# ChristophReich1996/Semantic_Pyramid_for_Image_Generation

Measured on AMD Instinct MI355X. Metric: images/sec full G+D train step, 256x256, bs/GPU=20, higher is better.
Workload: dtype bf16

## Files before the change

### include/sempyr.h

```cpp
#ifndef SEMPYR_H
#define SEMPYR_H
#include <stdint.h>

#ifdef __cplusplus
extern "C" {
#endif

#define SP_VERSION 1

typedef void* sp_stream_t;

enum sp_status { SP_OK = 0, SP_ERR_INVALID = -1, SP_ERR_LAUNCH = -2, SP_ERR_UNSUPPORTED = -3 };
enum sp_dtype { SP_F32 = 0, SP_BF16 = 1, SP_F8 = 2 ,
                SP_F16 = 3 ,
                SP_F8_F16 = 4  };
enum sp_act { SP_ACT_NONE = 0, SP_ACT_LRELU = 1, SP_ACT_RELU = 2, SP_ACT_TANH = 3 };

int sp_version(void);

enum { SP_TUNE_CONV_TALL = 0, SP_TUNE_IGEMM_DMA = 1, SP_TUNE_WGRAD_ROWS = 2, SP_TUNE_DETERMINISTIC = 3,
       SP_TUNE_SPLITK_TARGET = 4, SP_TUNE_SPLITK_MINSTEPS = 5, SP_TUNE_CONV1X1_DIRECT = 6, SP_TUNE_CONV_SHORT = 7,
       SP_TUNE_WGRAD9_BLOCKS = 8, SP_TUNE_WGRAD_BLOCKS = 9, SP_TUNE_WGRAD_MINSTEPS = 10, SP_TUNE_WGRAD_SMALL_M = 11,
       SP_TUNE_WGRAD_K1_TILE64 = 12, SP_TUNE_WGRAD_ROWS_THIN = 13, SP_TUNE_WGRAD_ROWS_BLOCKS = 14, SP_TUNE_WGRAD_ROWS_SLABS = 15,
       SP_TUNE_CONV_STAGGER = 16, SP_TUNE_CONV1X1_SPLITK = 17, SP_TUNE_WGRAD1X1 = 18, SP_TUNE_CONV_CIN8 = 19, SP_TUNE_CONV_THINCO = 20, SP_TUNE_CONV_PP = 21, SP_TUNE_CONV_PP_PRIO = 22, SP_TUNE_WGRAD_PP = 23, SP_TUNE_BN_ITERS = 24, SP_TUNE_IGEMM_TILE = 25, SP_TUNE_CONV_PPW = 26, SP_TUNE_LINEAR_KS = 27, SP_TUNE_CONV_PP_SPLIT = 28, SP_TUNE_PAIRSET_SEGMENTS = 29, SP_TUNE_COUNT = 30 };
int sp_set_tuning(int32_t key, int32_t value);
const char* sp_last_error_string(void);
const char* sp_last_route(void);

typedef struct sp_conv_params {
    const void* x;
    const void* w;
    const float* bias;
    void* y;
    const void* res1;
    const void* res2;
    const void* mask_src;
    float mask_neg_slope;
    int32_t n, h, w_, cin_p, cout, ldy, ksize, act, dtype;
    void* workspace;
    int64_t workspace_bytes;
    int32_t pool2;
    int32_t in_up2;
    const float* x_scale;
    const float* w_scale;
    void* y8;
    const float* y8_inv_scale;
    float* y8_amax;
    const float* img_scale;
    int32_t img_split;
    int32_t reserved_;
    int64_t split_pix_;
    const void* tail_w;
    const float* tail_bias;
    void* tail_y;
    int32_t tail_cout, tail_act, tail_ld, reserved2_;
    uint32_t* pool_idx;
    int32_t* split_sync;
} sp_conv_params;
#define SP_CONV_SPLIT_SYNC_BYTES 8192
int sp_conv2d_igemm(const sp_conv_params* p, sp_stream_t stream);
int sp_conv2d_workspace(int32_t n, int32_t h, int32_t w_, int32_t cin_p, int32_t cout, int32_t ksize, int32_t dtype,
                        int64_t* bytes_out);
int sp_conv2d_route(const sp_conv_params* p, const char** route);

int sp_conv2d_wgrad(const void* x, const void* dy, float* dw, int32_t n, int32_t h, int32_t w_,
                    int32_t cin_p, int32_t cout, int32_t ld_dy, int32_t ksize, int32_t dtype,
                    sp_stream_t stream);

int sp_conv2d_wgrad_fused(const void* x, const void* dy, float* dw, float* dbias, const void* w_packed, float* dot,
                          float* workspace, int64_t workspace_floats, int32_t n, int32_t h, int32_t w_, int32_t cin_p,
                          int32_t cout, int32_t ld_dy, int32_t ksize, int32_t dtype, sp_stream_t stream);
int sp_conv2d_wgrad_accum(const void* x, const void* dy, float* dw, float* dbias, float* workspace, int64_t workspace_floats,
                          int32_t n, int32_t h, int32_t w_, int32_t cin_p, int32_t cout, int32_t ld_dy, int32_t ksize,
                          int32_t dtype, sp_stream_t stream);
int sp_conv2d_wgrad_accum_pooled(const void* x, const void* dy, float* dw, float* dbias, float* workspace, int64_t workspace_floats,
                                 int32_t n, int32_t h, int32_t w_, int32_t cin_p, int32_t cout, int32_t ld_dy, int32_t ksize,
                                 int32_t dtype, sp_stream_t stream);
int sp_conv2d_wgrad_workspace(int32_t n, int32_t h, int32_t w_, int32_t cin_p, int32_t cout, int32_t ksize,
                              int32_t dtype, int64_t* floats_out);
int sp_conv2d_wgrad_accum_pair(const void* x, const void* dy, float* dw_a, float* dbias_a, float* dw_b, float* dbias_b, float* workspace,
                               int64_t workspace_floats, int32_t n, int32_t split, int32_t h, int32_t w_, int32_t cin_p, int32_t cout,
                               int32_t ld_dy, int32_t ksize, int32_t dy_pooled, int32_t dtype, sp_stream_t stream);
int sp_conv2d_wgrad_route(int32_t n, int32_t split, int32_t h, int32_t w_, int32_t cin_p, int32_t cout, int32_t ld_dy, int32_t ksize,
                          int32_t dy_pooled, int32_t want_dbias, int64_t workspace_floats, int32_t dtype, const char** route);
int sp_wgrad_reduce_defer(int32_t on);
int sp_wgrad_reduce_flush(int32_t run, sp_stream_t stream);
int sp_wgrad_reduce_pending(void);

int sp_linear_fwd(const void* x, int32_t ldx, const void* w_packed, int32_t kp, const float* bias,
                  const void* res, void* y, int32_t ldy, int32_t batch, int32_t k, int32_t n, int32_t act,
                  int32_t dtype, sp_stream_t stream);
int sp_linear_workspace(int32_t batch, int32_t k, int32_t n, int32_t dtype, int64_t* floats_out);
int sp_linear_fwd_ws(const void* x, int32_t ldx, const void* w_packed, int32_t kp, const float* bias,
                     const void* res, void* y, int32_t ldy, int32_t batch, int32_t k, int32_t n, int32_t act,
                     int32_t dtype, float* scratch, sp_stream_t stream);
int sp_linear_wgrad(const void* x, int32_t ldx, const void* dy, int32_t ld_dy, float* dw, int32_t kp,
                    float* dbias, int32_t batch, int32_t k, int32_t n, int32_t dtype, sp_stream_t stream);

typedef struct sp_sn_layer {
    const float* w;
    float* u;
    float* v;
    int64_t scratch_off;
    int64_t part_off;
    int64_t fwd_off;
    int64_t dgrad_off;
    int32_t rows, cols, cin, taps, cin_p, cout_p, kind, pack_block0;
} sp_sn_layer;
int sp_sn_forward(const sp_sn_layer* table_dev, int32_t n_layers, int32_t max_rows, int32_t max_cols,
                  int64_t max_pack_elems, float* scratch, int64_t scratch_floats, void* pack_arena,
                  int32_t power_iter, int32_t dtype, int32_t pack_blocks, sp_stream_t stream);
int sp_sn_pair_scales(const sp_sn_layer* table_dev, int32_t n_layers, const float* scratch_a, const float* scratch_b, float* out,
                      sp_stream_t stream);
typedef struct sp_sn_bwd_layer {
    const float* w;
    int64_t dw_off, dot_off, scratch_off, grad_off;
    int32_t rows, cols, cin, taps, cin_p, plain;
    int32_t db_off, bias_off;
} sp_sn_bwd_layer;
int sp_sn_backward_batched(const sp_sn_bwd_layer* table_dev, int32_t n_layers, int64_t max_elems, float* arena,
                           const float* scratch, float* grads, const float* accumulate_from, float* bias_grads,
                           float* dot_partials, sp_stream_t stream);
int sp_sn_backward_batched_scaled(const sp_sn_bwd_layer* table_dev, int32_t n_layers, int64_t max_elems, float* arena,
                                  const float* scratch, float* grads, const float* accumulate_from, float* bias_grads,
                                  float* dot_partials, float grad_scale, sp_stream_t stream);
int sp_sn_backward_batched_dscaled(const sp_sn_bwd_layer* table_dev, int32_t n_layers, int64_t max_elems, float* arena,
                                   const float* scratch, float* grads, const float* accumulate_from, float* bias_grads,
                                   float* dot_partials, const float* grad_scale_dev, sp_stream_t stream);

int sp_pack_weight(const float* w, int32_t rows, int32_t cols, int32_t cin, int32_t taps, int32_t cin_p,
                   int32_t cout_p, int32_t chw_c, int32_t chw_hw, void* fwd, void* dgrad, int32_t dtype,
                   sp_stream_t stream);
int sp_sn_backward(const float* dwsn, const float* w_orig, const float* layer_scratch, int32_t rows, int32_t cols,
                   int32_t cin, int32_t taps, int32_t cin_p, int32_t plain, float* dot_tmp, int32_t dot_ready,
                   float* grad, sp_stream_t stream);

int sp_bn_stats(const void* x, int32_t n, int64_t hw, int32_t c, float* partials, float eps, float momentum,
                float* running_mean, float* running_var, int32_t training, float* mean_out, float* invstd_out,
                int32_t dtype, sp_stream_t stream);
int sp_bn_apply(const void* x, void* y, int32_t n, int64_t hw, int32_t c, const float* mean, const float* invstd,
                const float* gamma, const float* beta, const float* emb, const int64_t* cls, int32_t act,
                int32_t dtype, sp_stream_t stream);
int sp_bn_stats_pair(const void* x, int32_t n, int32_t split, int64_t hw, int32_t c, float* partials, float eps, float momentum,
                     float* running_mean, float* running_var, int32_t first_group, float* mean2, float* invstd2, int32_t dtype,
                     sp_stream_t stream);
int sp_bn_apply_pair(const void* x, void* y, int32_t n, int32_t split, int64_t hw, int32_t c, const float* mean2, const float* invstd2,
                     const float* gamma, const float* beta, const float* emb, const int64_t* cls, int32_t act, int32_t dtype,
                     sp_stream_t stream);
int sp_bn_apply_upsample2_pair(const void* x, void* y, int32_t n, int32_t split, int32_t h, int32_t w_, int32_t c, const float* mean2,
                               const float* invstd2, const float* gamma, const float* beta, const float* emb, const int64_t* cls,
                               int32_t act, int32_t dtype, sp_stream_t stream);
int sp_bn_apply_upsample2(const void* x, void* y, int32_t n, int32_t h, int32_t w_, int32_t c, const float* mean,
                          const float* invstd, const float* gamma, const float* beta, const float* emb,
                          const int64_t* cls, int32_t act, int32_t dtype, sp_stream_t stream);
int sp_bn_backward(const void* dy, const void* x, void* dx, int32_t n, int64_t hw, int32_t c, const float* mean,
                   const float* invstd, const float* gamma, const float* beta, const float* emb, const int64_t* cls,
                   int32_t act, float* partials, float* c_tmp, float* dgamma, float* dbeta, float* demb,
                   int32_t num_classes, int32_t dtype, sp_stream_t stream);

int sp_bn_stats_up2(const void* x, int32_t n, int32_t h, int32_t w_, int32_t c, float* partials, float eps, float momentum,
                    float* running_mean, float* running_var, float* mean_out, float* invstd_out, int32_t dtype, sp_stream_t stream);
int sp_bn_apply_up2(const void* x, void* y, int32_t n, int32_t h, int32_t w_, int32_t c, const float* mean, const float* invstd,
                    const float* gamma, const float* beta, const float* emb, const int64_t* cls, int32_t act, int32_t dtype,
                    sp_stream_t stream);
int sp_bn_backward_up2(const void* dy, const void* x, void* du, int32_t n, int32_t h, int32_t w_, int32_t c, const float* mean,
                       const float* invstd, const float* gamma, const float* beta, const float* emb, const int64_t* cls,
                       int32_t act, float* partials, float* c_tmp, float* dgamma, float* dbeta, float* demb, int32_t num_classes,
                       int32_t dtype, sp_stream_t stream);

int sp_avgpool2_fwd(const void* x, void* y, void* y_act, int32_t act, int32_t n, int32_t h, int32_t w_, int32_t c,
                    int32_t dtype, sp_stream_t stream);
int sp_avgpool2_bwd(const void* dy, void* dx, int32_t n, int32_t h, int32_t w_, int32_t c, int32_t dtype,
                    sp_stream_t stream);
int sp_act_avgpool2_fwd(const void* x, void* y_act, void* y_pool, int32_t act, int32_t n, int32_t h, int32_t w_, int32_t c,
                        int32_t dtype, sp_stream_t stream);
int sp_act_avgpool2_bwd(const void* d_act, const void* d_pool, const void* x, void* dx, int32_t act, int32_t n, int32_t h,
                        int32_t w_, int32_t c, int32_t dtype, sp_stream_t stream);
int sp_maxpool2_fwd(const void* x, void* y, int32_t n, int32_t h, int32_t w_, int32_t c, int32_t relu, int32_t dtype,
                    sp_stream_t stream);
int sp_maxpool2_bwd(const void* dy, const void* x, void* dx, int32_t n, int32_t h, int32_t w_, int32_t c,
                    int32_t relu, int32_t dtype, sp_stream_t stream);
int sp_maxpool2_bwd_idx(const void* dy, const void* y, const uint32_t* idx, void* dx, int32_t n, int32_t h, int32_t w_, int32_t c,
                        int32_t dtype, sp_stream_t stream);
int sp_adaptive_avgpool_fwd(const void* x, void* y, int32_t n, int32_t h, int32_t w_, int32_t c, int32_t oh,
                            int32_t ow, int32_t act_in, int32_t dtype, sp_stream_t stream);
int sp_adaptive_avgpool_bwd(const void* dy, const void* x, void* dx, int32_t n, int32_t h, int32_t w_, int32_t c,
                            int32_t oh, int32_t ow, int32_t act_in, int32_t dtype, sp_stream_t stream);
int sp_upsample2_fwd(const void* x, void* y, int32_t n, int32_t h, int32_t w_, int32_t c, int32_t dtype,
                     sp_stream_t stream);
int sp_upsample2_bwd(const void* dy, void* dx, int32_t n, int32_t h, int32_t w_, int32_t c, int32_t dtype,
                     sp_stream_t stream);

int sp_attention_bwd_slabs(int32_t n, int32_t nk, int32_t d, int32_t dv, int32_t dtype, int64_t* slabs_out);
int sp_attention_fwd(const void* q, const void* k, const void* v, void* o, float* lse, int32_t batch, int32_t n,
                     int32_t nk, int32_t d, int32_t dv, int32_t dtype, sp_stream_t stream);
int sp_attention_bwd(const void* q, const void* k, const void* v, const void* dout, const float* lse, void* dq,
                     float* dk_f32, float* dv_f32, void* dk, void* dv_out, int32_t batch, int32_t n, int32_t nk,
                     int32_t d, int32_t dv, int32_t dtype, sp_stream_t stream);
int sp_attention_route(int32_t n, int32_t nk, int32_t d, int32_t dv, int32_t dtype, const char** fwd, const char** bwd);

int sp_ingest_image(const void* src, int32_t src_dtype, int64_t sn, int64_t sc, int64_t sh, int64_t sw, void* dst,
                    int32_t n, int32_t c, int32_t h, int32_t w_, int32_t cp, const float* scale3,
                    const float* shift3, int32_t dtype, sp_stream_t stream);
int sp_ingest_image_bwd(const void* dy, int32_t cp, void* dsrc, int32_t c, int64_t pixels, const float* scale3,
                        int32_t dtype, sp_stream_t stream);
enum { SP_AUG_COLOR = 1, SP_AUG_TRANSLATION = 2, SP_AUG_CUTOUT = 4 };
int sp_augment_slices(int32_t h, int32_t w_, int32_t backward, int64_t* slices_out);
int sp_augment_ingest(const void* src, int32_t src_dtype, int64_t sn, int64_t sc, int64_t sh, int64_t sw, void* dst,
                      int32_t n, int32_t h, int32_t w_, int32_t cp, const float* u, int32_t policy, float* partials,
                      int32_t dtype, sp_stream_t stream);
int sp_augment_ingest_bwd(const void* dy, int32_t cp, void* dsrc, int32_t n, int32_t h, int32_t w_, const float* u,
                          int32_t policy, float* partials, int32_t dtype, sp_stream_t stream);
int sp_augment_ingest_gated(const void* src, int32_t src_dtype, int64_t sn, int64_t sc, int64_t sh, int64_t sw, void* dst,
                            int32_t n, int32_t h, int32_t w_, int32_t cp, const float* u, int32_t policy, float* partials,
                            const float* p_dev, int32_t dtype, sp_stream_t stream);
int sp_augment_ingest_bwd_gated(const void* dy, int32_t cp, void* dsrc, int32_t n, int32_t h, int32_t w_, const float* u,
                                int32_t policy, float* partials, const float* p_dev, int32_t dtype, sp_stream_t stream);
int sp_ada_observe(const float* pred, int64_t numel, float threshold, void* state, sp_stream_t stream);
int sp_ada_adjust(void* state, int32_t interval, float target, float step, sp_stream_t stream);
int sp_apa_select(const void* real, int32_t real_dtype, int64_t rn, int64_t rc, int64_t rh, int64_t rw,
                  const void* fake, int32_t fake_dtype, int64_t fn, int64_t fc, int64_t fh, int64_t fw,
                  float* dst, int32_t n, int32_t h, int32_t w_,
                  const float* w_u, const float* p_dev, int32_t dtype, sp_stream_t stream);
enum { SP_GEOM_XFLIP = 1, SP_GEOM_ROT90 = 2, SP_GEOM_SCALE = 4, SP_GEOM_ROTATE = 8 };
int sp_augment_geom_slices(int32_t h, int32_t w_, int32_t backward, int64_t* slices_out);
int sp_augment_geom_decode(const float* u, const float* v, int32_t n, int32_t h, int32_t w_, int32_t policy, int32_t geom,
                           float* table, sp_stream_t stream);
int sp_augment_geom_ingest(const void* src, int32_t src_dtype, int64_t sn, int64_t sc, int64_t sh, int64_t sw, void* dst,
                           int32_t n, int32_t h, int32_t w_, int32_t cp, const float* u, int32_t policy, const float* table,
                           float* partials, const float* p_dev, int32_t dtype, sp_stream_t stream);
int sp_augment_geom_ingest_bwd(const void* dy, int32_t cp, void* dsrc, int32_t n, int32_t h, int32_t w_, const float* u,
                               int32_t policy, const float* table, float* partials, const float* p_dev, int32_t dtype,
                               sp_stream_t stream);
enum { SP_CMAT_BRIGHTNESS = 1, SP_CMAT_CONTRAST = 2, SP_CMAT_LUMAFLIP = 4, SP_CMAT_HUE = 8, SP_CMAT_SATURATION = 16 };
int sp_augment_cmat_decode(const float* z, int32_t n, int32_t cmat, float* ctable, sp_stream_t stream);
int sp_augment_cmat_ingest(const void* src, int32_t src_dtype, int64_t sn, int64_t sc, int64_t sh, int64_t sw, void* dst,
                           int32_t n, int32_t h, int32_t w_, int32_t cp, const float* u, int32_t policy, const float* table,
                           const float* ctable, float* partials, const float* p_dev, int32_t dtype, sp_stream_t stream);
int sp_augment_cmat_ingest_bwd(const void* dy, int32_t cp, void* dsrc, int32_t n, int32_t h, int32_t w_, const float* u,
                               int32_t policy, const float* table, const float* ctable, float* partials, const float* p_dev,
                               int32_t dtype, sp_stream_t stream);
int sp_mask_concat(const void* feat, const float* mask, void* out, int64_t pixels, int32_t c, int32_t cp,
                   int32_t dtype, sp_stream_t stream);
int sp_mask_mul_2d(const void* feat, int32_t ldf, const float* mask, void* out, int32_t ldo, int32_t batch,
                   int32_t k, int32_t dtype, sp_stream_t stream);
int sp_act_fwd(const void* x, void* y, int64_t numel, int32_t act, int32_t dtype, sp_stream_t stream);
int sp_act_bwd(const void* dy, const void* y, void* dz, int64_t pixels, int32_t c, int32_t cp, int32_t act,
               int32_t dtype, sp_stream_t stream);
int sp_scale_add(const void* a, const void* b, const float* g, void* y, int64_t numel, int32_t dtype,
                 sp_stream_t stream);
int sp_rescale_bias(const void* x, void* y, int64_t rows, int32_t c, int32_t ldx, int32_t ldy, const float* bias, const float* sig_a,
                    const float* sig_b, int32_t dtype, sp_stream_t stream);
int sp_scale_add_bwd(const void* dy, const void* a, const float* g, void* da, float* dg, float* partials, int64_t numel,
                     int32_t dtype, sp_stream_t stream);
int sp_permute_chw_hwc(const void* src, void* dst, int32_t batch, int32_t c, int32_t hw, int32_t to_hwc,
                       int32_t dtype, sp_stream_t stream);
int sp_channel_sum(const void* x, int32_t ld, int64_t pixels, int32_t c, float* out, float* partials, int32_t dtype,
                   sp_stream_t stream);
int sp_f64_to_f32(const double* src, float* dst, int32_t n, sp_stream_t stream);

int sp_dhead_fwd(const void* x, int32_t ldx, const float* emb_sn, const int64_t* cls, const float* wc,
                 const float* bc, float* pred, int32_t batch, int32_t f, int32_t dtype, sp_stream_t stream);
int sp_dhead_bwd(const float* dpred, const void* x, int32_t ldx, const float* emb_sn, const int64_t* cls,
                 const float* wc, void* dx, int32_t lddx, float* demb, int32_t num_classes, float* dwc, float* dbc,
                 float* scratch, int32_t batch, int32_t f, int32_t dtype, sp_stream_t stream);
int sp_sqerr_loss_fwd(const float* p, int64_t numel, float target, double* acc_tmp, float* loss, sp_stream_t stream);
int sp_sqerr_loss_bwd(const float* p, int64_t numel, float target, const float* gout, float* dp, sp_stream_t stream);
int sp_rec_loss_fwd(const void* real, int32_t ld_real, const void* fake, int32_t ld_fake, const float* mask,
                    int32_t n, int32_t h, int32_t w_, int32_t c, double* acc, int32_t dtype, sp_stream_t stream);
int sp_rec_loss_bwd(const void* real, int32_t ld_real, const void* fake, int32_t ld_fake, const float* mask,
                    const float* gout, void* dfake, int32_t ld_dfake, int32_t n, int32_t h, int32_t w_, int32_t c,
                    int32_t dtype, sp_stream_t stream);
int sp_div_loss_fwd(const void* img, int64_t half_elems, const float* z, int64_t half_z, double* acc_tmp,
                    float* out2, int32_t dtype, sp_stream_t stream);
int sp_div_loss_bwd(const void* img, int64_t half_elems, const float* fwd_out2, const float* gout, void* dimg,
                    int32_t dtype, sp_stream_t stream);
typedef struct sp_rec_level {
    const void* real; const void* fake; const float* mask;
    void* dfake;
    int32_t ld_real, ld_fake, ld_dfake, n, h, w_, c, reserved_;
} sp_rec_level;
int sp_rec_loss_fwd_levels(const sp_rec_level* levels, int32_t n_levels, double* acc, float* loss, float weight,
                           int32_t dtype, sp_stream_t stream);
int sp_rec_loss_bwd_levels(const sp_rec_level* levels, int32_t n_levels, const float* gout, float weight,
                           int32_t dtype, sp_stream_t stream);
int sp_div_loss_fwd_w(const void* img, int64_t half_elems, const float* z, int64_t half_z, double* acc,
                      float* out2, float weight, int32_t dtype, sp_stream_t stream);

int sp_gan_loss_fwd(const float* p, int64_t numel, int32_t kind, int32_t role, float* loss, sp_stream_t stream);
int sp_gan_loss_bwd(const float* p, int64_t numel, int32_t kind, int32_t role, const float* gout, float* dp, sp_stream_t stream);
int sp_lecam_fwd(const float* pred_real, const float* pred_fake, int64_t numel, float weight, float decay, int32_t start,
                 int32_t rectified, void* state, float* reg, sp_stream_t stream);
int sp_lecam_bwd(const float* pred_real, const float* pred_fake, int64_t numel, float weight, int32_t rectified, const void* state,
                 const float* gout, float* dpred_real, float* dpred_fake, sp_stream_t stream);

int sp_quantize_fp8(const void* x, void* q, int64_t numel, const float* inv_scale, float* amax, int32_t dtype, sp_stream_t stream);
int sp_pack_weight_fp8(const float* w, int32_t cout, int32_t cin, int32_t cin_p, void* out, float* w_scale, sp_stream_t stream);
int sp_fp8_update_scales(float* amax, float* scale, float* inv_scale, int32_t n, float margin, sp_stream_t stream);

int sp_minmax_normalize(const float* x, float* y, int32_t batch, int32_t channels, int64_t hw, float lo, float hi, float eps,
                        int32_t per_channel, sp_stream_t stream);

int sp_training_masks(float* m128, float* m64, float* m32, float* m16, float* m8, float* m4096, float* m365,
                      int32_t batch, uint64_t seed, float p_random_mask, sp_stream_t stream);

typedef struct sp_adam_chunk {
    float* p;
    const float* g;
    float* m;
    float* v;
    int32_t n;
    float step_size;
    float inv_sqrt_bc2;
    float reserved;
} sp_adam_chunk;
int sp_adam_multi(const sp_adam_chunk* chunks_dev, int32_t n_chunks, double beta1, double beta2, double eps,
                  double weight_decay, sp_stream_t stream);

int sp_scale_f32(float* x, int64_t numel, float factor, sp_stream_t stream);
int sp_scale_f32_dev(float* x, int64_t numel, const float* factor_dev, sp_stream_t stream);

int sp_check_finite(const float* x, int64_t numel, float* found, sp_stream_t stream);
int sp_adam_multi_guarded(const sp_adam_chunk* chunks_dev, int32_t n_chunks, double beta1, double beta2, double eps,
                          double weight_decay, const float* skip_if_nonzero, sp_stream_t stream);
int sp_loss_scale_update(float* state, float growth, float backoff, int32_t interval, sp_stream_t stream);

int sp_grad_sqnorm_multi(const sp_adam_chunk* chunks_dev, int32_t n_chunks, double* partials, sp_stream_t stream);
int sp_grad_clip_finalize(const double* partials, int32_t n_partials, double max_norm, float* state, sp_stream_t stream);
int sp_adam_multi_clipped(const sp_adam_chunk* chunks_dev, int32_t n_chunks, double beta1, double beta2, double eps,
                          double weight_decay, const float* skip_if_nonzero, const float* clip_state, sp_stream_t stream);

typedef struct sp_ema_chunk {
    float* avg;
    float* p;
    int32_t n;
    int32_t reserved;
} sp_ema_chunk;
int sp_ema_multi(const sp_ema_chunk* chunks_dev, int32_t n_chunks, float one_minus_decay, const float* skip_if_nonzero,
                 sp_stream_t stream);
int sp_swap_multi(const sp_ema_chunk* chunks_dev, int32_t n_chunks, sp_stream_t stream);

typedef struct sp_conv_general_params {
    int32_t struct_bytes;
    int32_t dtype;
    const void* x;
    const void* w;
    const float* bias;
    void* y;
    int32_t n, h, w_, cin_p, ldx, cout, ldy, kh, kw, stride_h, stride_w, pad_h, pad_w, act;
} sp_conv_general_params;
int sp_conv2d_general(const sp_conv_general_params* p, sp_stream_t stream);
int sp_maxpool3s2_fwd(const void* x, int32_t ldx, void* y, int32_t ldy, int32_t n, int32_t h, int32_t w_, int32_t c, int32_t dtype,
                      sp_stream_t stream);
int sp_avgpool3s1_fwd(const void* x, void* y, int32_t n, int32_t h, int32_t w_, int32_t c, int32_t dtype, sp_stream_t stream);
int sp_inception_prep(const float* x, float* minmax, void* y, int32_t n, int32_t c, int32_t h, int32_t w_, int32_t oh, int32_t ow,
                      int32_t cp, int32_t dtype, sp_stream_t stream);
int sp_global_avgpool_f32(const void* x, float* y, int32_t n, int32_t hw, int32_t c, int32_t dtype, sp_stream_t stream);


int sp_pairset_workspace(int32_t na, int32_t nb, int32_t d, int32_t k, int64_t* bytes);
int sp_pairset_knn(const float* a, int32_t na, int32_t lda, const float* b, int32_t nb, int32_t ldb, int32_t d, int32_t k,
                   int32_t same, float* radius, void* workspace, int64_t workspace_bytes, sp_stream_t stream);
int sp_pairset_cover(const float* a, int32_t na, int32_t lda, const float* b, int32_t nb, int32_t ldb, int32_t d,
                     const float* rad_a, const float* rad_b, int32_t* row_count, int32_t* col_count, float* row_min,
                     float* col_min, void* workspace, int64_t workspace_bytes, sp_stream_t stream);
int sp_pairset_poly3(const float* a, int32_t src_a, int32_t lda, const int32_t* idx_a, const float* b, int32_t src_b, int32_t ldb,
                     const int32_t* idx_b, int32_t d, int32_t subsets, int32_t m, int32_t skip_diag, double* out,
                     void* workspace, int64_t workspace_bytes, sp_stream_t stream);


int sp_pairset_softmax_workspace(int32_t n, int32_t classes, int32_t d, int32_t splits, int64_t* bytes);
int sp_pairset_lse(const float* a, int32_t n, int32_t lda, const float* w, int32_t classes, int32_t ldw, const float* bias, int32_t d,
                   double* lse, double* h, void* workspace, int64_t workspace_bytes, sp_stream_t stream);
int sp_pairset_softmax_colsum(const float* a, int32_t n, int32_t lda, const float* w, int32_t classes, int32_t ldw, const float* bias,
                              int32_t d, const double* lse, const double* h, int32_t splits, double* colsum, double* kl,
                              void* workspace, int64_t workspace_bytes, sp_stream_t stream);

#ifdef __cplusplus
}
#endif
#endif
```

### semantic_pyramid_for_image_generation_amd/_lib.py

```python
from __future__ import annotations

import ctypes
import os
import re
from typing import Dict, List, Tuple

_HERE = os.path.dirname(os.path.abspath(__file__))
HEADER = os.path.join(os.path.dirname(_HERE), "include", "sempyr.h")
LIB_PATH = os.environ.get("SEMPYR_LIB") or os.path.join(_HERE, "libsempyr.so")

SP_F32, SP_BF16, SP_F8, SP_F16, SP_F8_F16 = 0, 1, 2, 3, 4
ACT_NONE, ACT_LRELU, ACT_RELU, ACT_TANH = 0, 1, 2, 3

TUNE_KEYS = {"SP_CONV_TALL": 0, "SP_IGEMM_DMA": 1, "SP_WGRAD_ROWS": 2, "SP_DETERMINISTIC": 3, "SP_SPLITK_TARGET": 4,
             "SP_SPLITK_MINSTEPS": 5, "SP_CONV1X1_DIRECT": 6, "SP_CONV_SHORT": 7, "SP_WGRAD9_BLOCKS": 8, "SP_WGRAD_BLOCKS": 9,
             "SP_WGRAD_MINSTEPS": 10, "SP_WGRAD_SMALL_M": 11, "SP_WGRAD_K1_TILE64": 12, "SP_WGRAD_ROWS_THIN": 13,
             "SP_WGRAD_ROWS_BLOCKS": 14, "SP_WGRAD_ROWS_SLABS": 15, "SP_CONV_STAGGER": 16, "SP_CONV1X1_SPLITK": 17, "SP_WGRAD1X1": 18, "SP_CONV_CIN8": 19, "SP_CONV_THINCO": 20,
             "SP_CONV_PP": 21, "SP_CONV_PP_PRIO": 22, "SP_WGRAD_PP": 23, "SP_BN_ITERS": 24, "SP_IGEMM_TILE": 25, "SP_CONV_PPW": 26, "SP_LINEAR_KS": 27, "SP_CONV_PP_SPLIT": 28, "SP_PAIRSET_SEGMENTS": 29}


SP_CONV_SPLIT_SYNC_BYTES = 8192


class SpConvParams(ctypes.Structure):
    _fields_ = [("x", ctypes.c_void_p), ("w", ctypes.c_void_p), ("bias", ctypes.c_void_p), ("y", ctypes.c_void_p),
                ("res1", ctypes.c_void_p), ("res2", ctypes.c_void_p), ("mask_src", ctypes.c_void_p),
                ("mask_neg_slope", ctypes.c_float),
                ("n", ctypes.c_int32), ("h", ctypes.c_int32), ("w_", ctypes.c_int32), ("cin_p", ctypes.c_int32),
                ("cout", ctypes.c_int32), ("ldy", ctypes.c_int32), ("ksize", ctypes.c_int32), ("act", ctypes.c_int32),
                ("dtype", ctypes.c_int32), ("workspace", ctypes.c_void_p), ("workspace_bytes", ctypes.c_int64),
                ("pool2", ctypes.c_int32), ("in_up2", ctypes.c_int32),
                ("x_scale", ctypes.c_void_p), ("w_scale", ctypes.c_void_p), ("y8", ctypes.c_void_p),
                ("y8_inv_scale", ctypes.c_void_p), ("y8_amax", ctypes.c_void_p),
                ("img_scale", ctypes.c_void_p), ("img_split", ctypes.c_int32), ("reserved_", ctypes.c_int32),
                ("split_pix_", ctypes.c_int64),
                ("tail_w", ctypes.c_void_p), ("tail_bias", ctypes.c_void_p), ("tail_y", ctypes.c_void_p),
                ("tail_cout", ctypes.c_int32), ("tail_act", ctypes.c_int32), ("tail_ld", ctypes.c_int32), ("reserved2_", ctypes.c_int32),
                ("pool_idx", ctypes.c_void_p), ("split_sync", ctypes.c_void_p)]


class SpConvGeneralParams(ctypes.Structure):
    _fields_ = [("struct_bytes", ctypes.c_int32), ("dtype", ctypes.c_int32),
                ("x", ctypes.c_void_p), ("w", ctypes.c_void_p), ("bias", ctypes.c_void_p), ("y", ctypes.c_void_p),
                ("n", ctypes.c_int32), ("h", ctypes.c_int32), ("w_", ctypes.c_int32), ("cin_p", ctypes.c_int32),
                ("ldx", ctypes.c_int32), ("cout", ctypes.c_int32), ("ldy", ctypes.c_int32), ("kh", ctypes.c_int32),
                ("kw", ctypes.c_int32), ("stride_h", ctypes.c_int32), ("stride_w", ctypes.c_int32), ("pad_h", ctypes.c_int32),
                ("pad_w", ctypes.c_int32), ("act", ctypes.c_int32)]

    def __init__(self, **kw):
        super().__init__(struct_bytes=ctypes.sizeof(SpConvGeneralParams), **kw)


class SpSnLayer(ctypes.Structure):
    _fields_ = [("w", ctypes.c_void_p), ("u", ctypes.c_void_p), ("v", ctypes.c_void_p),
                ("scratch_off", ctypes.c_int64), ("part_off", ctypes.c_int64), ("fwd_off", ctypes.c_int64),
                ("dgrad_off", ctypes.c_int64),
                ("rows", ctypes.c_int32), ("cols", ctypes.c_int32), ("cin", ctypes.c_int32), ("taps", ctypes.c_int32),
                ("cin_p", ctypes.c_int32), ("cout_p", ctypes.c_int32), ("kind", ctypes.c_int32),
                ("pack_block0", ctypes.c_int32)]


class SpSnBwdLayer(ctypes.Structure):
    _fields_ = [("w", ctypes.c_void_p), ("dw_off", ctypes.c_int64), ("dot_off", ctypes.c_int64),
                ("scratch_off", ctypes.c_int64), ("grad_off", ctypes.c_int64),
                ("rows", ctypes.c_int32), ("cols", ctypes.c_int32), ("cin", ctypes.c_int32), ("taps", ctypes.c_int32),
                ("cin_p", ctypes.c_int32), ("plain", ctypes.c_int32), ("db_off", ctypes.c_int32),
                ("bias_off", ctypes.c_int32)]


class SpRecLevel(ctypes.Structure):
    _fields_ = [("real", ctypes.c_void_p), ("fake", ctypes.c_void_p), ("mask", ctypes.c_void_p), ("dfake", ctypes.c_void_p),
                ("ld_real", ctypes.c_int32), ("ld_fake", ctypes.c_int32), ("ld_dfake", ctypes.c_int32), ("n", ctypes.c_int32),
                ("h", ctypes.c_int32), ("w_", ctypes.c_int32), ("c", ctypes.c_int32), ("reserved_", ctypes.c_int32)]


_CTYPE = {"int32_t": ctypes.c_int32, "int64_t": ctypes.c_int64, "float": ctypes.c_float, "double": ctypes.c_double, "int": ctypes.c_int,
          "sp_stream_t": ctypes.c_void_p, "uint64_t": ctypes.c_uint64}


def parse_header(path: str = HEADER) -> Dict[str, Tuple[object, List[object]]]:
    text = open(path).read()
    text = re.sub(r"/\*.*?\*/", "", text, flags=re.S)
    protos = {}
    for m in re.finditer(r"\b(int|const char\*)\s+(sp_\w+)\s*\(([^;{]*?)\)\s*;", text, flags=re.S):
        ret, name, args = m.group(1), m.group(2), m.group(3).strip()
        argtypes = []
        if args and args != "void":
            for a in args.split(","):
                a = " ".join(a.split())
                if "*" in a:
                    argtypes.append(ctypes.c_void_p)
                else:
                    ty = a.rsplit(" ", 1)[0].replace("const ", "").strip()
                    argtypes.append(_CTYPE[ty])
        protos[name] = (ctypes.c_char_p if "char" in ret else ctypes.c_int, argtypes)
    return protos


class SempyrError(RuntimeError):
    pass


_lib = None
_protos = None


def lib():
    global _lib, _protos
    if _lib is None:
        if not os.path.exists(LIB_PATH):
            raise SempyrError("libsempyr.so not found at %s - build it with __graft_entry__.build() "
                              "(semantic_pyramid_for_image_generation_amd/csrc/build.sh); there is no fallback path"
                              % LIB_PATH)
        handle = ctypes.CDLL(LIB_PATH)
        _protos = parse_header()
        for name, (ret, argtypes) in _protos.items():
            fn = getattr(handle, name)
            fn.restype = ret
            fn.argtypes = argtypes
        for env_name, key in TUNE_KEYS.items():
            if os.environ.get(env_name) not in (None, ""):
                handle.sp_set_tuning(key, int(os.environ[env_name]))
        _lib = handle
    return _lib


def conv_route(p: SpConvParams) -> str:
    out = ctypes.c_char_p()
    call("sp_conv2d_route", ctypes.byref(p), ctypes.byref(out))
    return out.value.decode()


def wgrad_route(n, split, h, w, cin_p, cout, ld_dy, ksize, dy_pooled, want_dbias, workspace_floats, dtype) -> str:
    out = ctypes.c_char_p()
    call("sp_conv2d_wgrad_route", n, split, h, w, cin_p, cout, ld_dy, ksize, int(dy_pooled), int(want_dbias), workspace_floats, dtype, ctypes.byref(out))
    return out.value.decode()


def attention_route(n, nk, d, dv, dtype):
    fwd, bwd = ctypes.c_char_p(), ctypes.c_char_p()
    call("sp_attention_route", n, nk, d, dv, dtype, ctypes.byref(fwd), ctypes.byref(bwd))
    return fwd.value.decode(), bwd.value.decode()


def call(name: str, *args) -> None:
    rc = getattr(lib(), name)(*args)
    if rc != 0:
        raise SempyrError("%s failed (%d): %s" % (name, rc, lib().sp_last_error_string().decode()))
```

### semantic_pyramid_for_image_generation_amd/csrc/attention.hip

```cpp
#include "common.h"

namespace {


template <typename T, int TQ>
__global__ __launch_bounds__(256) void attn_fwd_kernel(const T* __restrict__ q, const T* __restrict__ k, const T* __restrict__ v,
                                                       T* __restrict__ o, float* __restrict__ lse, int N, int NK, int D, int DV) {
    extern __shared__ __attribute__((aligned(16))) float sm[];
    float* ks = sm;
    float* qs = ks + NK * (D + 1);
    float* S = qs + TQ * D;
    float* vs = S + TQ * NK;
    const int tid = threadIdx.x, lane = tid & 63, wave = tid >> 6;
    const int b = blockIdx.y, q0 = blockIdx.x * TQ;
    const T* kb = k + (long)b * NK * D;
    const T* vb = v + (long)b * NK * DV;
    const T* qb = q + ((long)b * N + q0) * D;
    for (int e = tid; e < NK * D; e += 256) ks[(e / D) * (D + 1) + e % D] = Elem<T>::ld(kb + e);
    for (int e = tid; e < TQ * D; e += 256) qs[e] = (q0 + e / D < N) ? Elem<T>::ld(qb + e) : 0.f;
    __syncthreads();
    for (int j = tid; j < NK; j += 256) {
        const float* kr = ks + j * (D + 1);
        for (int qi = 0; qi < TQ; ++qi) {
            float s = 0.f;
            for (int d = 0; d < D; ++d) s += qs[qi * D + d] * kr[d];
            S[qi * NK + j] = s;
        }
    }
    __syncthreads();
    for (int qi = wave; qi < TQ; qi += 4) {
        float m = -INFINITY;
        for (int j = lane; j < NK; j += 64) m = fmaxf(m, S[qi * NK + j]);
        m = wave_max(m);
        float sum = 0.f;
        for (int j = lane; j < NK; j += 64) { const float e = expf(S[qi * NK + j] - m); S[qi * NK + j] = e; sum += e; }
        sum = wave_sum(sum);
        const float inv = 1.f / sum;
        for (int j = lane; j < NK; j += 64) S[qi * NK + j] *= inv;
        if (lane == 0 && q0 + qi < N) lse[(long)b * N + q0 + qi] = m + logf(sum);
    }
    const int cpar = DV < 256 ? DV : 256;
    const int qpar = 256 / cpar;
    const int qph = tid / cpar;
    const int c = tid % cpar;
    const int nq = (TQ + qpar - 1) / qpar;
    float acc[TQ];
#pragma unroll
    for (int i = 0; i < TQ; ++i) acc[i] = 0.f;
    for (int j0 = 0; j0 < NK; j0 += 32) {
        __syncthreads();
        for (int e = tid; e < 32 * DV; e += 256) vs[e] = (j0 + e / DV < NK) ? Elem<T>::ld(vb + (long)j0 * DV + e) : 0.f;
        __syncthreads();
        if (qph < qpar) {
#pragma unroll 4
            for (int jj = 0; jj < 32; ++jj) {
                const float vv = vs[jj * DV + c];
#pragma unroll
                for (int i = 0; i < TQ; ++i)
                    if (i < nq) acc[i] += S[(qph + i * qpar) * NK + j0 + jj] * vv;
            }
        }
    }
    if (qph < qpar) {
#pragma unroll
        for (int i = 0; i < TQ; ++i) {
            const int qi = qph + i * qpar;
            if (i < nq && qi < TQ && q0 + qi < N) Elem<T>::st(o + ((long)b * N + q0 + qi) * DV + c, acc[i]);
        }
    }
}

template <typename T, int TQ>
__global__ __launch_bounds__(256) void attn_bwd_kernel(const T* __restrict__ q, const T* __restrict__ k, const T* __restrict__ v,
                                                       const T* __restrict__ dout, const float* __restrict__ lse,
                                                       T* __restrict__ dq, float* __restrict__ dk, float* __restrict__ dv,
                                                       int N, int NK, int D, int DV) {
    extern __shared__ __attribute__((aligned(16))) float sm[];
    float* ks = sm;
    float* qs = ks + NK * (D + 1);
    float* dos = qs + TQ * D;
    float* P = dos + TQ * DV;
    float* red = P + TQ * NK;
    float* vt = red + TQ * 4;
    const int tid = threadIdx.x, lane = tid & 63, wave = tid >> 6;
    const int b = blockIdx.y, q0 = blockIdx.x * TQ;
    const T* kb = k + (long)b * NK * D;
    const T* vb = v + (long)b * NK * DV;
    for (int e = tid; e < NK * D; e += 256) ks[(e / D) * (D + 1) + e % D] = Elem<T>::ld(kb + e);
    for (int e = tid; e < TQ * D; e += 256) qs[e] = (q0 + e / D < N) ? Elem<T>::ld(q + ((long)b * N + q0) * D + e) : 0.f;
    for (int e = tid; e < TQ * DV; e += 256) dos[e] = (q0 + e / DV < N) ? Elem<T>::ld(dout + ((long)b * N + q0) * DV + e) : 0.f;
    __syncthreads();
    const int j = tid;
    const bool jl = j < NK;
    float p[TQ], dp[TQ];
#pragma unroll
    for (int qi = 0; qi < TQ; ++qi) { p[qi] = 0.f; dp[qi] = 0.f; }
    if (jl) {
        const float* kr = ks + j * (D + 1);
#pragma unroll
        for (int qi = 0; qi < TQ; ++qi) {
            float s = 0.f;
            for (int d = 0; d < D; ++d) s += qs[qi * D + d] * kr[d];
            p[qi] = (q0 + qi < N) ? expf(s - lse[(long)b * N + q0 + qi]) : 0.f;
        }
    }
    for (int c0 = 0; c0 < DV; c0 += 32) {
        __syncthreads();
        for (int e = tid; e < NK * 32; e += 256) {
            const int jj = e >> 5, cc = e & 31;
            vt[cc * (NK + 1) + jj] = (c0 + cc < DV) ? Elem<T>::ld(vb + (long)jj * DV + c0 + cc) : 0.f;
        }
        __syncthreads();
        if (jl) {
#pragma unroll 4
            for (int cc = 0; cc < 32; ++cc) {
                if (c0 + cc >= DV) break;
                const float vv = vt[cc * (NK + 1) + j];
#pragma unroll
                for (int qi = 0; qi < TQ; ++qi) dp[qi] += dos[qi * DV + c0 + cc] * vv;
            }
        }
    }
    if (jl) {
#pragma unroll
        for (int qi = 0; qi < TQ; ++qi) P[qi * NK + j] = p[qi];
    }
    __syncthreads();
    {
        const int cpar = DV < 256 ? DV : 256, jpar = 256 / cpar;
        const int c = tid % cpar, jph = tid / cpar;
        if (jph < jpar) {
            float dcol[TQ];
#pragma unroll
            for (int qi = 0; qi < TQ; ++qi) dcol[qi] = dos[qi * DV + c];
            for (int jj = jph; jj < NK; jj += jpar) {
                float a = 0.f;
#pragma unroll
                for (int qi = 0; qi < TQ; ++qi) a += P[qi * NK + jj] * dcol[qi];
                dv[((long)blockIdx.x * gridDim.y + b) * NK * DV + (long)jj * DV + c] = a;
            }
        }
    }
#pragma unroll
    for (int qi = 0; qi < TQ; ++qi) {
        const float w = wave_sum(p[qi] * dp[qi]);
        if (lane == 0) red[qi * 4 + wave] = w;
    }
    __syncthreads();
    if (jl) {
#pragma unroll
        for (int qi = 0; qi < TQ; ++qi) {
            const float dr = red[qi * 4] + red[qi * 4 + 1] + red[qi * 4 + 2] + red[qi * 4 + 3];
            const float ds = p[qi] * (dp[qi] - dr);
            P[qi * NK + j] = ds;
            p[qi] = ds;
        }
        for (int d = 0; d < D; ++d) {
            float a = 0.f;
#pragma unroll
            for (int qi = 0; qi < TQ; ++qi) a += p[qi] * qs[qi * D + d];
            dk[((long)blockIdx.x * gridDim.y + b) * NK * D + (long)j * D + d] = a;
        }
    }
    __syncthreads();
    for (int e = tid; e < TQ * D; e += 256) {
        const int qi = e / D, d = e - qi * D;
        float a = 0.f;
        for (int jj = 0; jj < NK; ++jj) a += P[qi * NK + jj] * ks[jj * (D + 1) + d];
        if (q0 + qi < N) Elem<T>::st(dq + ((long)b * N + q0 + qi) * D + d, a);
    }
}


constexpr int AM_NKMAX = 256;
__global__ __launch_bounds__(256) void attn_fwd_mfma_kernel(const bf16* __restrict__ q, const bf16* __restrict__ k,
                                                            const bf16* __restrict__ v, bf16* __restrict__ o, float* __restrict__ lse,
                                                            int N, int NK, int D, int DV) {
    extern __shared__ __attribute__((aligned(16))) char vsm[];
    const int PV = DV * 2 + 32;
    const int tid = threadIdx.x, lane = tid & 63, wave = tid >> 6;
    const int b = blockIdx.y;
    const int q0 = blockIdx.x * 64 + wave * 16;
    const bf16* kb = k + (long)b * NK * D;
    const bf16* vb = v + (long)b * NK * DV;
    const int cpr = DV / 8;
    for (int e = tid; e < NK * cpr; e += 256) {
        const int row = e / cpr, c = e - row * cpr;
        *reinterpret_cast<uint4*>(vsm + row * PV + c * 16) = *reinterpret_cast<const uint4*>(vb + (long)row * DV + c * 8);
    }
    const int i16 = lane & 15, g = lane >> 4;
    const int qrow = min(q0 + i16, N - 1);
    const bf16* qp = q + ((long)b * N + qrow) * D + g * 8;
    f32x4_t sfr[AM_NKMAX / 16];
    const int nf = NK / 16;
#pragma unroll
    for (int f = 0; f < AM_NKMAX / 16; ++f) sfr[f] = f32x4_t{0.f, 0.f, 0.f, 0.f};
    for (int d0 = 0; d0 < D; d0 += 32) {
        const uint4 qv = *reinterpret_cast<const uint4*>(qp + d0);
#pragma unroll
        for (int f = 0; f < AM_NKMAX / 16; ++f) {
            if (f < nf) {
                const uint4 kv = *reinterpret_cast<const uint4*>(kb + (long)(f * 16 + i16) * D + d0 + g * 8);
                sfr[f] = __builtin_amdgcn_mfma_f32_16x16x32_bf16(__builtin_bit_cast(bf16x8_t, kv), __builtin_bit_cast(bf16x8_t, qv), sfr[f], 0, 0, 0);
            }
        }
    }
    float m = -INFINITY;
#pragma unroll
    for (int f = 0; f < AM_NKMAX / 16; ++f)
        if (f < nf) m = fmaxf(fmaxf(fmaxf(m, sfr[f][0]), fmaxf(sfr[f][1], sfr[f][2])), sfr[f][3]);
    m = fmaxf(m, __shfl_xor(m, 16, 64));
    m = fmaxf(m, __shfl_xor(m, 32, 64));
    float sum = 0.f;
#pragma unroll
    for (int f = 0; f < AM_NKMAX / 16; ++f)
        if (f < nf) {
#pragma unroll
            for (int r = 0; r < 4; ++r) { const float e = __expf(sfr[f][r] - m); sfr[f][r] = e; sum += e; }
        }
    sum += __shfl_xor(sum, 16, 64);
    sum += __shfl_xor(sum, 32, 64);
    const float inv = 1.f / sum;
    if (g == 0 && q0 + i16 < N) lse[(long)b * N + q0 + i16] = m + __logf(sum);
    __syncthreads();
    f32x4_t oacc[16];
    const int ncb = DV / 16;
#pragma unroll
    for (int cb = 0; cb < 16; ++cb) oacc[cb] = f32x4_t{0.f, 0.f, 0.f, 0.f};
#pragma unroll
    for (int t = 0; t < AM_NKMAX / 32; ++t) {
        if (t * 32 < NK) {
            uint4 pb;
            pb.x = f32x2_to_bf16x2(sfr[2 * t][0] * inv, sfr[2 * t][1] * inv);
            pb.y = f32x2_to_bf16x2(sfr[2 * t][2] * inv, sfr[2 * t][3] * inv);
            pb.z = f32x2_to_bf16x2(sfr[2 * t + 1][0] * inv, sfr[2 * t + 1][1] * inv);
            pb.w = f32x2_to_bf16x2(sfr[2 * t + 1][2] * inv, sfr[2 * t + 1][3] * inv);
            const char* vrow = vsm + (t * 32 + g * 4 + (i16 >> 2)) * PV + (i16 & 3) * 8;
#pragma unroll
            for (int cb = 0; cb < 16; ++cb) {
                if (cb < ncb) {
                    s16x4_t lo = __builtin_amdgcn_ds_read_tr16_b64_v4i16((__attribute__((address_space(3))) s16x4_t*)(vrow + cb * 32));
                    s16x4_t hi = __builtin_amdgcn_ds_read_tr16_b64_v4i16((__attribute__((address_space(3))) s16x4_t*)(vrow + cb * 32 + 16 * PV));
                    uint2 l2 = __builtin_bit_cast(uint2, lo), h2 = __builtin_bit_cast(uint2, hi);
                    const uint4 va = make_uint4(l2.x, l2.y, h2.x, h2.y);
                    oacc[cb] = __builtin_amdgcn_mfma_f32_16x16x32_bf16(__builtin_bit_cast(bf16x8_t, va), __builtin_bit_cast(bf16x8_t, pb), oacc[cb], 0, 0, 0);
                }
            }
        }
    }
    if (q0 + i16 < N) {
        bf16* op = o + ((long)b * N + q0 + i16) * DV + g * 4;
#pragma unroll
        for (int cb = 0; cb < 16; ++cb)
            if (cb < ncb) {
                const float t4[4] = {oacc[cb][0], oacc[cb][1], oacc[cb][2], oacc[cb][3]};
                Elem<bf16>::st4(op + cb * 16, t4);
            }
    }
}

constexpr int AB_QB = 64;
__device__ __forceinline__ uint4 tr_pair(const char* p, int hi_off) {
    s16x4_t lo = __builtin_amdgcn_ds_read_tr16_b64_v4i16((__attribute__((address_space(3))) s16x4_t*)(p));
    s16x4_t hi = __builtin_amdgcn_ds_read_tr16_b64_v4i16((__attribute__((address_space(3))) s16x4_t*)(p + hi_off));
    const uint2 l2 = __builtin_bit_cast(uint2, lo), h2 = __builtin_bit_cast(uint2, hi);
    return make_uint4(l2.x, l2.y, h2.x, h2.y);
}
__device__ __forceinline__ uint4 pack8(const f32x4_t& a, const f32x4_t& b) {
    uint4 r;
    r.x = f32x2_to_bf16x2(a[0], a[1]);
    r.y = f32x2_to_bf16x2(a[2], a[3]);
    r.z = f32x2_to_bf16x2(b[0], b[1]);
    r.w = f32x2_to_bf16x2(b[2], b[3]);
    return r;
}

__global__ __launch_bounds__(256) void attn_bwd_mfma_kernel(const bf16* __restrict__ q, const bf16* __restrict__ k,
                                                            const bf16* __restrict__ v, const bf16* __restrict__ dout,
                                                            const float* __restrict__ lse, bf16* __restrict__ dq,
                                                            float* __restrict__ dk, float* __restrict__ dv, int N, int NK, int D, int DV) {
    extern __shared__ __attribute__((aligned(16))) char bsm[];
    const int PK = D * 2 + 32, PDO = DV * 2 + 32, PP = NK * 2 + 32;
    char* Ksm = bsm;
    char* Qsm = Ksm + NK * PK;
    char* dOsm = Qsm + AB_QB * PK;
    char* Psm = dOsm + AB_QB * PDO;
    char* dSsm = Psm + AB_QB * PP;
    const int PVL = DV * 2 + 16;
    const bool v_in_lds = NK * PVL <= 2 * AB_QB * PP;
    const int tid = threadIdx.x, lane = tid & 63, wave = tid >> 6;
    const int b = blockIdx.y, qb0 = blockIdx.x * AB_QB;
    const bf16* kb = k + (long)b * NK * D;
    const bf16* vb = v + (long)b * NK * DV;
    float* dk_slab = dk + (long)blockIdx.x * gridDim.y * NK * D;
    float* dv_slab = dv + (long)blockIdx.x * gridDim.y * NK * DV;
    {
        const int cpr = D / 8;
        for (int e = tid; e < NK * cpr; e += 256) {
            const int row = e / cpr, c = e - row * cpr;
            *reinterpret_cast<uint4*>(Ksm + row * PK + c * 16) = *reinterpret_cast<const uint4*>(kb + (long)row * D + c * 8);
        }
        for (int e = tid; e < AB_QB * cpr; e += 256) {
            const int row = e / cpr, c = e - row * cpr;
            uint4 val = make_uint4(0, 0, 0, 0);
            if (qb0 + row < N) val = *reinterpret_cast<const uint4*>(q + ((long)b * N + qb0 + row) * D + c * 8);
            *reinterpret_cast<uint4*>(Qsm + row * PK + c * 16) = val;
        }
        const int cpo = DV / 8;
        for (int e = tid; e < AB_QB * cpo; e += 256) {
            const int row = e / cpo, c = e - row * cpo;
            uint4 val = make_uint4(0, 0, 0, 0);
            if (qb0 + row < N) val = *reinterpret_cast<const uint4*>(dout + ((long)b * N + qb0 + row) * DV + c * 8);
            *reinterpret_cast<uint4*>(dOsm + row * PDO + c * 16) = val;
        }
        if (v_in_lds) {
            for (int e = tid; e < NK * cpo; e += 256) {
                const int row = e / cpo, c = e - row * cpo;
                *reinterpret_cast<uint4*>(Psm + row * PVL + c * 16) = *reinterpret_cast<const uint4*>(vb + (long)row * DV + c * 8);
            }
        }
    }
    __syncthreads();
    const int i16 = lane & 15, g = lane >> 4;
    const int ql = wave * 16 + i16;
    const bool q_ok = qb0 + ql < N;
    const int nf = NK / 16;
    f32x4_t pfr[AM_NKMAX / 16], dpf[AM_NKMAX / 16];
#pragma unroll
    for (int f = 0; f < AM_NKMAX / 16; ++f) { pfr[f] = f32x4_t{0.f, 0.f, 0.f, 0.f}; dpf[f] = f32x4_t{0.f, 0.f, 0.f, 0.f}; }
    for (int d0 = 0; d0 < D; d0 += 32) {
        const uint4 qv = *reinterpret_cast<const uint4*>(Qsm + ql * PK + (d0 + g * 8) * 2);
#pragma unroll
        for (int f = 0; f < AM_NKMAX / 16; ++f)
            if (f < nf) {
                const uint4 kv = *reinterpret_cast<const uint4*>(Ksm + (f * 16 + i16) * PK + (d0 + g * 8) * 2);
                pfr[f] = __builtin_amdgcn_mfma_f32_16x16x32_bf16(__builtin_bit_cast(bf16x8_t, kv), __builtin_bit_cast(bf16x8_t, qv), pfr[f], 0, 0, 0);
            }
    }
    for (int c0 = 0; c0 < DV; c0 += 32) {
        const uint4 dov = *reinterpret_cast<const uint4*>(dOsm + ql * PDO + (c0 + g * 8) * 2);
#pragma unroll
        for (int f = 0; f < AM_NKMAX / 16; ++f)
            if (f < nf) {
                const uint4 vv = v_in_lds ? *reinterpret_cast<const uint4*>(Psm + (f * 16 + i16) * PVL + (c0 + g * 8) * 2)
                                          : *reinterpret_cast<const uint4*>(vb + (long)(f * 16 + i16) * DV + c0 + g * 8);
                dpf[f] = __builtin_amdgcn_mfma_f32_16x16x32_bf16(__builtin_bit_cast(bf16x8_t, vv), __builtin_bit_cast(bf16x8_t, dov), dpf[f], 0, 0, 0);
            }
    }
    const float l = q_ok ? lse[(long)b * N + qb0 + ql] : 0.f;
    float drow = 0.f;
#pragma unroll
    for (int f = 0; f < AM_NKMAX / 16; ++f)
        if (f < nf) {
#pragma unroll
            for (int r = 0; r < 4; ++r) {
                const float pv = q_ok ? __expf(pfr[f][r] - l) : 0.f;
                pfr[f][r] = pv;
                drow += pv * dpf[f][r];
            }
        }
    drow += __shfl_xor(drow, 16, 64);
    drow += __shfl_xor(drow, 32, 64);
#pragma unroll
    for (int f = 0; f < AM_NKMAX / 16; ++f)
        if (f < nf) {
#pragma unroll
            for (int r = 0; r < 4; ++r) dpf[f][r] = pfr[f][r] * (dpf[f][r] - drow);
        }
    {
        f32x4_t dqa[4];
        const int ndb = D / 16;
#pragma unroll
        for (int db = 0; db < 4; ++db) dqa[db] = f32x4_t{0.f, 0.f, 0.f, 0.f};
#pragma unroll
        for (int t = 0; t < AM_NKMAX / 32; ++t)
            if (t * 32 < NK) {
                const uint4 sb = pack8(dpf[2 * t], dpf[2 * t + 1]);
                const char* krow = Ksm + (t * 32 + g * 4 + (i16 >> 2)) * PK + (i16 & 3) * 8;
#pragma unroll
                for (int db = 0; db < 4; ++db)
                    if (db < ndb) {
                        const uint4 ka = tr_pair(krow + db * 32, 16 * PK);
                        dqa[db] = __builtin_amdgcn_mfma_f32_16x16x32_bf16(__builtin_bit_cast(bf16x8_t, ka), __builtin_bit_cast(bf16x8_t, sb), dqa[db], 0, 0, 0);
                    }
            }
        if (q_ok) {
            bf16* qp = dq + ((long)b * N + qb0 + ql) * D + g * 4;
#pragma unroll
            for (int db = 0; db < 4; ++db)
                if (db < ndb) {
                    const float t4[4] = {dqa[db][0], dqa[db][1], dqa[db][2], dqa[db][3]};
                    Elem<bf16>::st4(qp + db * 16, t4);
                }
        }
    }
    if (v_in_lds) __syncthreads();
#pragma unroll
    for (int f = 0; f < AM_NKMAX / 16; ++f)
        if (f < nf) {
            uint2 pw, sw;
            pw.x = f32x2_to_bf16x2(pfr[f][0], pfr[f][1]);
            pw.y = f32x2_to_bf16x2(pfr[f][2], pfr[f][3]);
            sw.x = f32x2_to_bf16x2(dpf[f][0], dpf[f][1]);
            sw.y = f32x2_to_bf16x2(dpf[f][2], dpf[f][3]);
            *reinterpret_cast<uint2*>(Psm + ql * PP + (f * 16 + g * 4) * 2) = pw;
            *reinterpret_cast<uint2*>(dSsm + ql * PP + (f * 16 + g * 4) * 2) = sw;
        }
    __syncthreads();
    const int rowsel = g * 4 + (i16 >> 2), colsel = (i16 & 3) * 8;
    for (int cb0 = 0; cb0 < DV / 16; cb0 += 8) {
        f32x4_t acc[4][8];
        const int ncb = min(8, DV / 16 - cb0);
#pragma unroll
        for (int a = 0; a < 4; ++a)
#pragma unroll
            for (int cb = 0; cb < 8; ++cb) acc[a][cb] = f32x4_t{0.f, 0.f, 0.f, 0.f};
#pragma unroll
        for (int t2 = 0; t2 < AB_QB / 32; ++t2) {
            uint4 pb[4];
#pragma unroll
            for (int a = 0; a < 4; ++a) {
                const int kf = wave + 4 * a;
                pb[a] = tr_pair(Psm + (t2 * 32 + rowsel) * PP + colsel + (kf < nf ? kf : 0) * 32, 16 * PP);
            }
#pragma unroll
            for (int cb = 0; cb < 8; ++cb)
                if (cb < ncb) {
                    const uint4 da = tr_pair(dOsm + (t2 * 32 + rowsel) * PDO + colsel + (cb0 + cb) * 32, 16 * PDO);
#pragma unroll
                    for (int a = 0; a < 4; ++a)
                        acc[a][cb] = __builtin_amdgcn_mfma_f32_16x16x32_bf16(__builtin_bit_cast(bf16x8_t, da), __builtin_bit_cast(bf16x8_t, pb[a]), acc[a][cb], 0, 0, 0);
                }
        }
#pragma unroll
        for (int a = 0; a < 4; ++a) {
            const int kf = wave + 4 * a;
            if (kf < nf) {
                float* dst = dv_slab + ((long)b * NK + kf * 16 + i16) * DV + cb0 * 16 + g * 4;
#pragma unroll
                for (int cb = 0; cb < 8; ++cb)
                    if (cb < ncb) *reinterpret_cast<float4*>(dst + cb * 16) = make_float4(acc[a][cb][0], acc[a][cb][1], acc[a][cb][2], acc[a][cb][3]);
            }
        }
    }
    {
        f32x4_t acc[4][4];
        const int ndb = D / 16;
#pragma unroll
        for (int a = 0; a < 4; ++a)
#pragma unroll
            for (int db = 0; db < 4; ++db) acc[a][db] = f32x4_t{0.f, 0.f, 0.f, 0.f};
#pragma unroll
        for (int t2 = 0; t2 < AB_QB / 32; ++t2) {
            uint4 sb[4];
#pragma unroll
            for (int a = 0; a < 4; ++a) {
                const int kf = wave + 4 * a;
                sb[a] = tr_pair(dSsm + (t2 * 32 + rowsel) * PP + colsel + (kf < nf ? kf : 0) * 32, 16 * PP);
            }
#pragma unroll
            for (int db = 0; db < 4; ++db)
                if (db < ndb) {
                    const uint4 qa = tr_pair(Qsm + (t2 * 32 + rowsel) * PK + colsel + db * 32, 16 * PK);
#pragma unroll
                    for (int a = 0; a < 4; ++a)
                        acc[a][db] = __builtin_amdgcn_mfma_f32_16x16x32_bf16(__builtin_bit_cast(bf16x8_t, qa), __builtin_bit_cast(bf16x8_t, sb[a]), acc[a][db], 0, 0, 0);
                }
        }
#pragma unroll
        for (int a = 0; a < 4; ++a) {
            const int kf = wave + 4 * a;
            if (kf < nf) {
                float* dst = dk_slab + ((long)b * NK + kf * 16 + i16) * D + g * 4;
#pragma unroll
                for (int db = 0; db < 4; ++db)
                    if (db < ndb) *reinterpret_cast<float4*>(dst + db * 16) = make_float4(acc[a][db][0], acc[a][db][1], acc[a][db][2], acc[a][db][3]);
            }
        }
    }
}

template <typename T>
__global__ void attn_reduce_kernel(const float* __restrict__ src, int nslabs, long n, T* __restrict__ dst) {
    for (long i = (long)blockIdx.x * 256 + threadIdx.x; i < n / 4; i += (long)gridDim.x * 256) {
        float4 a = reinterpret_cast<const float4*>(src)[i];
        for (int s = 1; s < nslabs; ++s) {
            const float4 t = reinterpret_cast<const float4*>(src + (long)s * n)[i];
            a.x += t.x; a.y += t.y; a.z += t.z; a.w += t.w;
        }
        const float o[4] = {a.x, a.y, a.z, a.w};
        Elem<T>::st4(dst + i * 4, o);
    }
}

template <typename T>
__global__ void cast_f32_kernel(const float* __restrict__ src, T* __restrict__ dst, long n) {
    for (long i = (long)blockIdx.x * 256 + threadIdx.x; i < n; i += (long)gridDim.x * 256) Elem<T>::st(dst + i, src[i]);
}

template <typename T, int TQ>
int launch_attn_tq(bool fwd, const void* q, const void* k, const void* v, void* o_or_dq, const void* dout, float* lse, float* dk,
                   float* dv, int B, int N, int NK, int D, int DV, hipStream_t s) {
    const int lds_f = (NK * (D + 1) + TQ * D + TQ * NK + 32 * DV) * 4;
    const int lds_b = (NK * (D + 1) + TQ * D + TQ * DV + TQ * NK + TQ * 4 + 32 * (NK + 1)) * 4;
    dim3 grid(sp_div_up(N, TQ), B);
    if (fwd) {
        if (const int rc = sp_lds_limit<attn_fwd_kernel<T, TQ>>(lds_f)) return rc;
        hipLaunchKernelGGL((attn_fwd_kernel<T, TQ>), grid, dim3(256), lds_f, s, (const T*)q, (const T*)k, (const T*)v, (T*)o_or_dq, lse, N, NK, D, DV);
    } else {
        if (const int rc = sp_lds_limit<attn_bwd_kernel<T, TQ>>(lds_b)) return rc;
        hipLaunchKernelGGL((attn_bwd_kernel<T, TQ>), grid, dim3(256), lds_b, s, (const T*)q, (const T*)k, (const T*)v, (const T*)dout, lse,
                           (T*)o_or_dq, dk, dv, N, NK, D, DV);
    }
    SP_LAUNCH_CHECK();
    return SP_OK;
}

inline int attn_valu_tq(int NK, int D, int DV) {
    const long lds_b32 = (long)(NK * (D + 1) + 32 * D + 32 * DV + 32 * NK + 32 * 4 + 32 * (NK + 1)) * 4;
    return lds_b32 <= 160 * 1024 ? 32 : 16;
}
inline bool attn_fwd_mfma_ok(int dtype, int nk, int d, int dv) {
    return dtype == SP_BF16 && d % 32 == 0 && dv % 16 == 0 && dv <= 256 && nk % 32 == 0;
}
inline bool attn_bwd_mfma_ok(int dtype, int nk, int d, int dv) {
    return dtype == SP_BF16 && (d == 32 || d == 64) && dv % 32 == 0 && dv <= 256 && nk % 32 == 0;
}
inline const char* attn_valu_name(int nk, int d, int dv) { return attn_valu_tq(nk, d, dv) == 32 ? "valu tq32" : "valu tq16"; }
template <typename T>
int launch_attn(bool fwd, const void* q, const void* k, const void* v, void* o_or_dq, const void* dout, float* lse, float* dk,
                float* dv, int B, int N, int NK, int D, int DV, hipStream_t s) {
    if (attn_valu_tq(NK, D, DV) == 32) return launch_attn_tq<T, 32>(fwd, q, k, v, o_or_dq, dout, lse, dk, dv, B, N, NK, D, DV, s);
    return launch_attn_tq<T, 16>(fwd, q, k, v, o_or_dq, dout, lse, dk, dv, B, N, NK, D, DV, s);
}

}

extern "C" int sp_attention_fwd(const void* q, const void* k, const void* v, void* o, float* lse, int32_t batch, int32_t n,
                                int32_t nk, int32_t d, int32_t dv, int32_t dtype, sp_stream_t stream) {
    SP_CHECK_ARG(q && k && v && o && lse, "sp_attention_fwd: null pointer");
    SP_CHECK_ARG(nk > 0 && nk <= 256 && d > 0 && d <= 64 && dv > 0 && dv <= 256, "sp_attention_fwd: unsupported extents nk=%d d=%d dv=%d", nk, d, dv);
    hipStream_t s = reinterpret_cast<hipStream_t>(stream);
    if (attn_fwd_mfma_ok(dtype, nk, d, dv)) {
        const int lds = nk * (dv * 2 + 32);
        if (const int rc = sp_lds_limit<attn_fwd_mfma_kernel>(lds)) return rc;
        hipLaunchKernelGGL(attn_fwd_mfma_kernel, dim3(sp_div_up(n, 64), batch), dim3(256), lds, s, (const bf16*)q, (const bf16*)k, (const bf16*)v,
                           (bf16*)o, lse, n, nk, d, dv);
        SP_LAUNCH_CHECK();
        return SP_OK;
    }
    return dtype == SP_F32 ? launch_attn<float>(true, q, k, v, o, nullptr, lse, nullptr, nullptr, batch, n, nk, d, dv, s)
                           : launch_attn<bf16>(true, q, k, v, o, nullptr, lse, nullptr, nullptr, batch, n, nk, d, dv, s);
}

extern "C" int sp_attention_bwd(const void* q, const void* k, const void* v, const void* dout, const float* lse, void* dq,
                                float* dk_f32, float* dv_f32, void* dk, void* dv_out, int32_t batch, int32_t n, int32_t nk,
                                int32_t d, int32_t dv, int32_t dtype, sp_stream_t stream) {
    SP_CHECK_ARG(q && k && v && dout && lse && dq && dk_f32 && dv_f32 && dk && dv_out, "sp_attention_bwd: null pointer");
    SP_CHECK_ARG(nk > 0 && nk <= 256 && d > 0 && d <= 64 && dv > 0 && dv <= 256, "sp_attention_bwd: unsupported extents nk=%d d=%d dv=%d", nk, d, dv);
    hipStream_t s = reinterpret_cast<hipStream_t>(stream);
    const long nkd = (long)batch * nk * d, nkv = (long)batch * nk * dv;
    if (attn_bwd_mfma_ok(dtype, nk, d, dv)) {
        const int nqb = sp_div_up(n, AB_QB);
        const int lds = nk * (d * 2 + 32) + AB_QB * (d * 2 + 32) + AB_QB * (dv * 2 + 32) + 2 * AB_QB * (nk * 2 + 32);
        if (const int rc = sp_lds_limit<attn_bwd_mfma_kernel>(lds)) return rc;
        hipLaunchKernelGGL(attn_bwd_mfma_kernel, dim3(nqb, batch), dim3(256), lds, s, (const bf16*)q, (const bf16*)k,
                           (const bf16*)v, (const bf16*)dout, lse, (bf16*)dq, dk_f32, dv_f32, n, nk, d, dv);
        hipLaunchKernelGGL(attn_reduce_kernel<bf16>, dim3(sp_div_up(nkd / 4, 256)), dim3(256), 0, s, dk_f32, nqb, nkd, (bf16*)dk);
        hipLaunchKernelGGL(attn_reduce_kernel<bf16>, dim3(sp_div_up(nkv / 4, 256)), dim3(256), 0, s, dv_f32, nqb, nkv, (bf16*)dv_out);
        SP_LAUNCH_CHECK();
        return SP_OK;
    }
    SP_CHECK_ARG(nkd % 4 == 0 && nkv % 4 == 0, "sp_attention_bwd: batch*nk*d and batch*nk*dv must be multiples of 4");
    const int nqb = sp_div_up(n, attn_valu_tq(nk, d, dv));
    int rc = dtype == SP_F32 ? launch_attn<float>(false, q, k, v, dq, dout, const_cast<float*>(lse), dk_f32, dv_f32, batch, n, nk, d, dv, s)
                             : launch_attn<bf16>(false, q, k, v, dq, dout, const_cast<float*>(lse), dk_f32, dv_f32, batch, n, nk, d, dv, s);
    if (rc != SP_OK) return rc;
    if (dtype == SP_F32) {
        hipLaunchKernelGGL(attn_reduce_kernel<float>, dim3(sp_div_up(nkd / 4, 256)), dim3(256), 0, s, dk_f32, nqb, nkd, (float*)dk);
        hipLaunchKernelGGL(attn_reduce_kernel<float>, dim3(sp_div_up(nkv / 4, 256)), dim3(256), 0, s, dv_f32, nqb, nkv, (float*)dv_out);
    } else {
        hipLaunchKernelGGL(attn_reduce_kernel<bf16>, dim3(sp_div_up(nkd / 4, 256)), dim3(256), 0, s, dk_f32, nqb, nkd, (bf16*)dk);
        hipLaunchKernelGGL(attn_reduce_kernel<bf16>, dim3(sp_div_up(nkv / 4, 256)), dim3(256), 0, s, dv_f32, nqb, nkv, (bf16*)dv_out);
    }
    SP_LAUNCH_CHECK();
    return SP_OK;
}

extern "C" int sp_attention_bwd_slabs(int32_t n, int32_t nk, int32_t d, int32_t dv, int32_t dtype, int64_t* slabs_out) {
    SP_CHECK_ARG(slabs_out && n > 0 && nk > 0 && d > 0 && dv > 0, "sp_attention_bwd_slabs: bad args");
    *slabs_out = attn_bwd_mfma_ok(dtype, nk, d, dv) ? sp_div_up(n, AB_QB) : sp_div_up(n, attn_valu_tq(nk, d, dv));
    return SP_OK;
}

extern "C" int sp_attention_route(int32_t n, int32_t nk, int32_t d, int32_t dv, int32_t dtype, const char** fwd, const char** bwd) {
    SP_CHECK_ARG(fwd != nullptr && bwd != nullptr, "sp_attention_route: null argument");
    SP_CHECK_ARG(dtype == SP_F32 || dtype == SP_BF16, "sp_attention_route: unsupported storage type %d", dtype);
    SP_CHECK_ARG(n > 0 && nk > 0 && nk <= 256 && d > 0 && d <= 64 && dv > 0 && dv <= 256, "sp_attention_route: unsupported extents n=%d nk=%d d=%d dv=%d", n, nk, d, dv);
    *fwd = attn_fwd_mfma_ok(dtype, nk, d, dv) ? "mfma" : attn_valu_name(nk, d, dv);
    *bwd = attn_bwd_mfma_ok(dtype, nk, d, dv) ? "mfma" : attn_valu_name(nk, d, dv);
    return SP_OK;
}
```

Before: 1322.

## Make attention blocks walk several query tiles, keeping K/V resident across tiles

The forward attention kernel now loops over several 64-row query tiles per block. K stays in registers when d=32 and V is staged into LDS once per block, so it is reused across tiles instead of reloaded per tile. A new backward kernel keeps K and V resident in LDS while walking query tiles, which cuts the number of fp32 dK/dV slabs. The two slab reductions are merged into one launch. The walk length is derived from the CU count and can be overridden by a new tuning key. Fewer blocks means less parallelism for small batches, and a cycle-counter timing variant of the old backward kernel is added behind a tuning flag.

Result: faster. 1339, median of 6 (+1.3%).

```diff
diff --git a/include/sempyr.h b/include/sempyr.h
--- a/include/sempyr.h
+++ b/include/sempyr.h
@@ -22,7 +22,7 @@
        SP_TUNE_SPLITK_TARGET = 4, SP_TUNE_SPLITK_MINSTEPS = 5, SP_TUNE_CONV1X1_DIRECT = 6, SP_TUNE_CONV_SHORT = 7,
        SP_TUNE_WGRAD9_BLOCKS = 8, SP_TUNE_WGRAD_BLOCKS = 9, SP_TUNE_WGRAD_MINSTEPS = 10, SP_TUNE_WGRAD_SMALL_M = 11,
        SP_TUNE_WGRAD_K1_TILE64 = 12, SP_TUNE_WGRAD_ROWS_THIN = 13, SP_TUNE_WGRAD_ROWS_BLOCKS = 14, SP_TUNE_WGRAD_ROWS_SLABS = 15,
-       SP_TUNE_CONV_STAGGER = 16, SP_TUNE_CONV1X1_SPLITK = 17, SP_TUNE_WGRAD1X1 = 18, SP_TUNE_CONV_CIN8 = 19, SP_TUNE_CONV_THINCO = 20, SP_TUNE_CONV_PP = 21, SP_TUNE_CONV_PP_PRIO = 22, SP_TUNE_WGRAD_PP = 23, SP_TUNE_BN_ITERS = 24, SP_TUNE_IGEMM_TILE = 25, SP_TUNE_CONV_PPW = 26, SP_TUNE_LINEAR_KS = 27, SP_TUNE_CONV_PP_SPLIT = 28, SP_TUNE_PAIRSET_SEGMENTS = 29, SP_TUNE_COUNT = 30 };
+       SP_TUNE_CONV_STAGGER = 16, SP_TUNE_CONV1X1_SPLITK = 17, SP_TUNE_WGRAD1X1 = 18, SP_TUNE_CONV_CIN8 = 19, SP_TUNE_CONV_THINCO = 20, SP_TUNE_CONV_PP = 21, SP_TUNE_CONV_PP_PRIO = 22, SP_TUNE_WGRAD_PP = 23, SP_TUNE_BN_ITERS = 24, SP_TUNE_IGEMM_TILE = 25, SP_TUNE_CONV_PPW = 26, SP_TUNE_LINEAR_KS = 27, SP_TUNE_CONV_PP_SPLIT = 28, SP_TUNE_PAIRSET_SEGMENTS = 29, SP_TUNE_ATTN_PIECES = 30, SP_TUNE_COUNT = 31 };
 int sp_set_tuning(int32_t key, int32_t value);
 const char* sp_last_error_string(void);
 const char* sp_last_route(void);
@@ -198,6 +198,8 @@
                      float* dk_f32, float* dv_f32, void* dk, void* dv_out, int32_t batch, int32_t n, int32_t nk,
                      int32_t d, int32_t dv, int32_t dtype, sp_stream_t stream);
 int sp_attention_route(int32_t n, int32_t nk, int32_t d, int32_t dv, int32_t dtype, const char** fwd, const char** bwd);
+int sp_attention_plan(int32_t batch, int32_t n, int32_t nk, int32_t d, int32_t dv, int32_t dtype, int32_t cus,
+                      int32_t* fwd_walk, int32_t* bwd_walk, int32_t* bwd_slabs);
 
 int sp_ingest_image(const void* src, int32_t src_dtype, int64_t sn, int64_t sc, int64_t sh, int64_t sw, void* dst,
                     int32_t n, int32_t c, int32_t h, int32_t w_, int32_t cp, const float* scale3,
diff --git a/semantic_pyramid_for_image_generation_amd/_lib.py b/semantic_pyramid_for_image_generation_amd/_lib.py
--- a/semantic_pyramid_for_image_generation_amd/_lib.py
+++ b/semantic_pyramid_for_image_generation_amd/_lib.py
@@ -16,7 +16,7 @@
              "SP_SPLITK_MINSTEPS": 5, "SP_CONV1X1_DIRECT": 6, "SP_CONV_SHORT": 7, "SP_WGRAD9_BLOCKS": 8, "SP_WGRAD_BLOCKS": 9,
              "SP_WGRAD_MINSTEPS": 10, "SP_WGRAD_SMALL_M": 11, "SP_WGRAD_K1_TILE64": 12, "SP_WGRAD_ROWS_THIN": 13,
              "SP_WGRAD_ROWS_BLOCKS": 14, "SP_WGRAD_ROWS_SLABS": 15, "SP_CONV_STAGGER": 16, "SP_CONV1X1_SPLITK": 17, "SP_WGRAD1X1": 18, "SP_CONV_CIN8": 19, "SP_CONV_THINCO": 20,
-             "SP_CONV_PP": 21, "SP_CONV_PP_PRIO": 22, "SP_WGRAD_PP": 23, "SP_BN_ITERS": 24, "SP_IGEMM_TILE": 25, "SP_CONV_PPW": 26, "SP_LINEAR_KS": 27, "SP_CONV_PP_SPLIT": 28, "SP_PAIRSET_SEGMENTS": 29}
+             "SP_CONV_PP": 21, "SP_CONV_PP_PRIO": 22, "SP_WGRAD_PP": 23, "SP_BN_ITERS": 24, "SP_IGEMM_TILE": 25, "SP_CONV_PPW": 26, "SP_LINEAR_KS": 27, "SP_CONV_PP_SPLIT": 28, "SP_PAIRSET_SEGMENTS": 29, "SP_ATTN_PIECES": 30}
 
 
 SP_CONV_SPLIT_SYNC_BYTES = 8192
diff --git a/semantic_pyramid_for_image_generation_amd/csrc/attention.hip b/semantic_pyramid_for_image_generation_amd/csrc/attention.hip
--- a/semantic_pyramid_for_image_generation_amd/csrc/attention.hip
+++ b/semantic_pyramid_for_image_generation_amd/csrc/attention.hip
@@ -173,93 +173,146 @@
 
 
 constexpr int AM_NKMAX = 256;
-__global__ __launch_bounds__(256) void attn_fwd_mfma_kernel(const bf16* __restrict__ q, const bf16* __restrict__ k,
-                                                            const bf16* __restrict__ v, bf16* __restrict__ o, float* __restrict__ lse,
-                                                            int N, int NK, int D, int DV) {
+constexpr int AB_QB = 64;
+
+template <int BATCH>
+__device__ __forceinline__ void stage_chunks(char* dst, int pitch, const bf16* __restrict__ src, int chunks, int live, int cpr, int tid) {
+    const uint4* s4 = reinterpret_cast<const uint4*>(src);
+    for (int e0 = tid; e0 < chunks; e0 += 256 * BATCH) {
+        uint4 r[BATCH];
+#pragma unroll
+        for (int i = 0; i < BATCH; ++i) r[i] = s4[min(e0 + i * 256, live - 1)];
+#pragma unroll
+        for (int i = 0; i < BATCH; ++i) {
+            const int e = e0 + i * 256;
+            if (e < chunks) {
+                const int row = e / cpr, c = e - row * cpr;
+                *reinterpret_cast<uint4*>(dst + row * pitch + c * 16) = e < live ? r[i] : make_uint4(0, 0, 0, 0);
+            }
+        }
+    }
+}
+
+constexpr int ATTN_TIMING_BIT = 4096;
+inline int attn_walk(int batch, int nqb, int slots, int pieces) {
+    if (pieces >= ATTN_TIMING_BIT) pieces = -1;
+    if (pieces >= 0) return sp_div_up(nqb, pieces < 1 ? 1 : pieces > nqb ? nqb : pieces);
+    int r = 1;
+    while (r < nqb && (long)batch * sp_div_up(nqb, r) > slots) ++r;
+    return r;
+}
+inline int attn_cus() {
+    static const int cus = [] {
+        int dev = 0, n = 0;
+        if (hipGetDevice(&dev) != hipSuccess || hipDeviceGetAttribute(&n, hipDeviceAttributeMultiprocessorCount, dev) != hipSuccess || n <= 0) {
+            (void)hipGetLastError();
+            n = 256;
+        }
+        return n;
+    }();
+    return cus;
+}
+inline int attn_fwd_lds(int nk, int dv) { return nk * (dv * 2 + 32); }
+inline int attn_fwd_slots(int cus, int nk, int dv) { return 2 * attn_fwd_lds(nk, dv) <= 160 * 1024 ? 2 * cus : cus; }
+
+template <bool KREG>
+__global__ __launch_bounds__(256, 2) void attn_fwd_mfma_kernel(const bf16* __restrict__ q, const bf16* __restrict__ k,
+                                                               const bf16* __restrict__ v, bf16* __restrict__ o, float* __restrict__ lse,
+                                                               int N, int NK, int D, int DV, int R) {
     extern __shared__ __attribute__((aligned(16))) char vsm[];
     const int PV = DV * 2 + 32;
     const int tid = threadIdx.x, lane = tid & 63, wave = tid >> 6;
     const int b = blockIdx.y;
-    const int q0 = blockIdx.x * 64 + wave * 16;
+    const int nqb = (N + AB_QB - 1) / AB_QB;
+    const int blk0 = blockIdx.x * R, nit = min(R, nqb - blk0);
     const bf16* kb = k + (long)b * NK * D;
     const bf16* vb = v + (long)b * NK * DV;
-    const int cpr = DV / 8;
-    for (int e = tid; e < NK * cpr; e += 256) {
-        const int row = e / cpr, c = e - row * cpr;
-        *reinterpret_cast<uint4*>(vsm + row * PV + c * 16) = *reinterpret_cast<const uint4*>(vb + (long)row * DV + c * 8);
-    }
     const int i16 = lane & 15, g = lane >> 4;
-    const int qrow = min(q0 + i16, N - 1);
-    const bf16* qp = q + ((long)b * N + qrow) * D + g * 8;
-    f32x4_t sfr[AM_NKMAX / 16];
     const int nf = NK / 16;
-#pragma unroll
-    for (int f = 0; f < AM_NKMAX / 16; ++f) sfr[f] = f32x4_t{0.f, 0.f, 0.f, 0.f};
-    for (int d0 = 0; d0 < D; d0 += 32) {
-        const uint4 qv = *reinterpret_cast<const uint4*>(qp + d0);
-#pragma unroll
-        for (int f = 0; f < AM_NKMAX / 16; ++f) {
+    const bf16* qimg = q + (long)b * N * D + g * 8;
+    uint4 qv0 = *reinterpret_cast<const uint4*>(qimg + (long)min(blk0 * AB_QB + wave * 16 + i16, N - 1) * D);
+    uint4 kfr[KREG ? AM_NKMAX / 16 : 1];
+    if constexpr (KREG) {
+#pragma unroll
+        for (int f = 0; f < AM_NKMAX / 16; ++f)
+            kfr[f] = *reinterpret_cast<const uint4*>(kb + (long)(min(f, nf - 1) * 16 + i16) * D + g * 8);
+    }
+    stage_chunks<8>(vsm, PV, vb, NK * (DV / 8), NK * (DV / 8), DV / 8, tid);
+    __syncthreads();
+    for (int it = 0; it < nit; ++it) {
+        const int q0 = (blk0 + it) * AB_QB + wave * 16;
+        const int qrow = min(q0 + i16, N - 1);
+        uint4 qv = qv0;
+        if (it + 1 < nit) qv0 = *reinterpret_cast<const uint4*>(qimg + (long)min(q0 + AB_QB + i16, N - 1) * D);
+        f32x4_t sfr[AM_NKMAX / 16];
+#pragma unroll
+        for (int f = 0; f < AM_NKMAX / 16; ++f) sfr[f] = f32x4_t{0.f, 0.f, 0.f, 0.f};
+        for (int d0 = 0; d0 < D; d0 += 32) {
+            if (d0 > 0) qv = *reinterpret_cast<const uint4*>(qimg + (long)qrow * D + d0);
+#pragma unroll
+            for (int f = 0; f < AM_NKMAX / 16; ++f) {
+                if (f < nf) {
+                    uint4 kv;
+                    if constexpr (KREG) kv = kfr[f];
+                    else kv = *reinterpret_cast<const uint4*>(kb + (long)(f * 16 + i16) * D + d0 + g * 8);
+                    sfr[f] = __builtin_amdgcn_mfma_f32_16x16x32_bf16(__builtin_bit_cast(bf16x8_t, kv), __builtin_bit_cast(bf16x8_t, qv), sfr[f], 0, 0, 0);
+                }
+            }
+        }
+        float m = -INFINITY;
+#pragma unroll
+        for (int f = 0; f < AM_NKMAX / 16; ++f)
+            if (f < nf) m = fmaxf(fmaxf(fmaxf(m, sfr[f][0]), fmaxf(sfr[f][1], sfr[f][2])), sfr[f][3]);
+        m = fmaxf(m, __shfl_xor(m, 16, 64));
+        m = fmaxf(m, __shfl_xor(m, 32, 64));
+        float sum = 0.f;
+#pragma unroll
+        for (int f = 0; f < AM_NKMAX / 16; ++f)
             if (f < nf) {
-                const uint4 kv = *reinterpret_cast<const uint4*>(kb + (long)(f * 16 + i16) * D + d0 + g * 8);
-                sfr[f] = __builtin_amdgcn_mfma_f32_16x16x32_bf16(__builtin_bit_cast(bf16x8_t, kv), __builtin_bit_cast(bf16x8_t, qv), sfr[f], 0, 0, 0);
-            }
-        }
-    }
-    float m = -INFINITY;
-#pragma unroll
-    for (int f = 0; f < AM_NKMAX / 16; ++f)
-        if (f < nf) m = fmaxf(fmaxf(fmaxf(m, sfr[f][0]), fmaxf(sfr[f][1], sfr[f][2])), sfr[f][3]);
-    m = fmaxf(m, __shfl_xor(m, 16, 64));
-    m = fmaxf(m, __shfl_xor(m, 32, 64));
-    float sum = 0.f;
-#pragma unroll
-    for (int f = 0; f < AM_NKMAX / 16; ++f)
-        if (f < nf) {
-#pragma unroll
-            for (int r = 0; r < 4; ++r) { const float e = __expf(sfr[f][r] - m); sfr[f][r] = e; sum += e; }
-        }
-    sum += __shfl_xor(sum, 16, 64);
-    sum += __shfl_xor(sum, 32, 64);
-    const float inv = 1.f / sum;
-    if (g == 0 && q0 + i16 < N) lse[(long)b * N + q0 + i16] = m + __logf(sum);
-    __syncthreads();
-    f32x4_t oacc[16];
-    const int ncb = DV / 16;
-#pragma unroll
-    for (int cb = 0; cb < 16; ++cb) oacc[cb] = f32x4_t{0.f, 0.f, 0.f, 0.f};
-#pragma unroll
-    for (int t = 0; t < AM_NKMAX / 32; ++t) {
-        if (t * 32 < NK) {
-            uint4 pb;
-            pb.x = f32x2_to_bf16x2(sfr[2 * t][0] * inv, sfr[2 * t][1] * inv);
-            pb.y = f32x2_to_bf16x2(sfr[2 * t][2] * inv, sfr[2 * t][3] * inv);
-            pb.z = f32x2_to_bf16x2(sfr[2 * t + 1][0] * inv, sfr[2 * t + 1][1] * inv);
-            pb.w = f32x2_to_bf16x2(sfr[2 * t + 1][2] * inv, sfr[2 * t + 1][3] * inv);
-            const char* vrow = vsm + (t * 32 + g * 4 + (i16 >> 2)) * PV + (i16 & 3) * 8;
-#pragma unroll
-            for (int cb = 0; cb < 16; ++cb) {
+#pragma unroll
+                for (int r = 0; r < 4; ++r) { const float e = __expf(sfr[f][r] - m); sfr[f][r] = e; sum += e; }
+            }
+        sum += __shfl_xor(sum, 16, 64);
+        sum += __shfl_xor(sum, 32, 64);
+        const float inv = 1.f / sum;
+        if (g == 0 && q0 + i16 < N) lse[(long)b * N + q0 + i16] = m + __logf(sum);
+        f32x4_t oacc[16];
+        const int ncb = DV / 16;
+#pragma unroll
+        for (int cb = 0; cb < 16; ++cb) oacc[cb] = f32x4_t{0.f, 0.f, 0.f, 0.f};
+#pragma unroll
+        for (int t = 0; t < AM_NKMAX / 32; ++t) {
+            if (t * 32 < NK) {
+                uint4 pb;
+                pb.x = f32x2_to_bf16x2(sfr[2 * t][0] * inv, sfr[2 * t][1] * inv);
+                pb.y = f32x2_to_bf16x2(sfr[2 * t][2] * inv, sfr[2 * t][3] * inv);
+                pb.z = f32x2_to_bf16x2(sfr[2 * t + 1][0] * inv, sfr[2 * t + 1][1] * inv);
+                pb.w = f32x2_to_bf16x2(sfr[2 * t + 1][2] * inv, sfr[2 * t + 1][3] * inv);
+                const char* vrow = vsm + (t * 32 + g * 4 + (i16 >> 2)) * PV + (i16 & 3) * 8;
+#pragma unroll
+                for (int cb = 0; cb < 16; ++cb) {
+                    if (cb < ncb) {
+                        s16x4_t lo = __builtin_amdgcn_ds_read_tr16_b64_v4i16((__attribute__((address_space(3))) s16x4_t*)(vrow + cb * 32));
+                        s16x4_t hi = __builtin_amdgcn_ds_read_tr16_b64_v4i16((__attribute__((address_space(3))) s16x4_t*)(vrow + cb * 32 + 16 * PV));
+                        uint2 l2 = __builtin_bit_cast(uint2, lo), h2 = __builtin_bit_cast(uint2, hi);
+                        const uint4 va = make_uint4(l2.x, l2.y, h2.x, h2.y);
+                        oacc[cb] = __builtin_amdgcn_mfma_f32_16x16x32_bf16(__builtin_bit_cast(bf16x8_t, va), __builtin_bit_cast(bf16x8_t, pb), oacc[cb], 0, 0, 0);
+                    }
+                }
+            }
+        }
+        if (q0 + i16 < N) {
+            bf16* op = o + ((long)b * N + q0 + i16) * DV + g * 4;
+#pragma unroll
+            for (int cb = 0; cb < 16; ++cb)
                 if (cb < ncb) {
-                    s16x4_t lo = __builtin_amdgcn_ds_read_tr16_b64_v4i16((__attribute__((address_space(3))) s16x4_t*)(vrow + cb * 32));
-                    s16x4_t hi = __builtin_amdgcn_ds_read_tr16_b64_v4i16((__attribute__((address_space(3))) s16x4_t*)(vrow + cb * 32 + 16 * PV));
-                    uint2 l2 = __builtin_bit_cast(uint2, lo), h2 = __builtin_bit_cast(uint2, hi);
-                    const uint4 va = make_uint4(l2.x, l2.y, h2.x, h2.y);
-                    oacc[cb] = __builtin_amdgcn_mfma_f32_16x16x32_bf16(__builtin_bit_cast(bf16x8_t, va), __builtin_bit_cast(bf16x8_t, pb), oacc[cb], 0, 0, 0);
-                }
-            }
-        }
-    }
-    if (q0 + i16 < N) {
-        bf16* op = o + ((long)b * N + q0 + i16) * DV + g * 4;
-#pragma unroll
-        for (int cb = 0; cb < 16; ++cb)
-            if (cb < ncb) {
-                const float t4[4] = {oacc[cb][0], oacc[cb][1], oacc[cb][2], oacc[cb][3]};
-                Elem<bf16>::st4(op + cb * 16, t4);
-            }
-    }
-}
-
-constexpr int AB_QB = 64;
+                    const float t4[4] = {oacc[cb][0], oacc[cb][1], oacc[cb][2], oacc[cb][3]};
+                    Elem<bf16>::st4(op + cb * 16, t4);
+                }
+        }
+    }
+}
+
 __device__ __forceinline__ uint4 tr_pair(const char* p, int hi_off) {
     s16x4_t lo = __builtin_amdgcn_ds_read_tr16_b64_v4i16((__attribute__((address_space(3))) s16x4_t*)(p));
     s16x4_t hi = __builtin_amdgcn_ds_read_tr16_b64_v4i16((__attribute__((address_space(3))) s16x4_t*)(p + hi_off));
@@ -275,6 +328,7 @@
     return r;
 }
 
+template <bool TIMING = false>
 __global__ __launch_bounds__(256) void attn_bwd_mfma_kernel(const bf16* __restrict__ q, const bf16* __restrict__ k,
                                                             const bf16* __restrict__ v, const bf16* __restrict__ dout,
                                                             const float* __restrict__ lse, bf16* __restrict__ dq,
@@ -294,6 +348,16 @@
     const bf16* vb = v + (long)b * NK * DV;
     float* dk_slab = dk + (long)blockIdx.x * gridDim.y * NK * D;
     float* dv_slab = dv + (long)blockIdx.x * gridDim.y * NK * DV;
+    unsigned long long tacc[6] = {0, 0, 0, 0, 0, 0};
+    unsigned long long tprev = 0;
+    auto stamp = [&](int i) {
+        if constexpr (TIMING) {
+            const unsigned long long t = __builtin_readcyclecounter();
+            tacc[i] += t - tprev;
+            tprev = t;
+        }
+    };
+    if constexpr (TIMING) tprev = __builtin_readcyclecounter();
     {
         const int cpr = D / 8;
         for (int e = tid; e < NK * cpr; e += 256) {
@@ -321,6 +385,7 @@
         }
     }
     __syncthreads();
+    stamp(0);
     const int i16 = lane & 15, g = lane >> 4;
     const int ql = wave * 16 + i16;
     const bool q_ok = qb0 + ql < N;
@@ -367,6 +432,7 @@
 #pragma unroll
             for (int r = 0; r < 4; ++r) dpf[f][r] = pfr[f][r] * (dpf[f][r] - drow);
         }
+    stamp(1);
     {
         f32x4_t dqa[4];
         const int ndb = D / 16;
@@ -394,6 +460,7 @@
                 }
         }
     }
+    stamp(2);
     if (v_in_lds) __syncthreads();
 #pragma unroll
     for (int f = 0; f < AM_NKMAX / 16; ++f)
@@ -407,6 +474,7 @@
             *reinterpret_cast<uint2*>(dSsm + ql * PP + (f * 16 + g * 4) * 2) = sw;
         }
     __syncthreads();
+    stamp(3);
     const int rowsel = g * 4 + (i16 >> 2), colsel = (i16 & 3) * 8;
     for (int cb0 = 0; cb0 < DV / 16; cb0 += 8) {
         f32x4_t acc[4][8];
@@ -443,6 +511,7 @@
             }
         }
     }
+    stamp(4);
     {
         f32x4_t acc[4][4];
         const int ndb = D / 16;
@@ -478,6 +547,241 @@
             }
         }
     }
+    if constexpr (TIMING) {
+        stamp(5);
+        __syncthreads();
+        if (lane == 0)
+            for (int i = 0; i < 6; ++i) dk_slab[(long)b * NK * D + wave * 8 + i] = (float)tacc[i];
+    }
+}
+
+inline int attn_bwd_res_lds(int nk, int d, int dv) {
+    return nk * (d * 2 + 32) + nk * (dv * 2 + 16) + AB_QB * (d * 2 + 32) + AB_QB * (dv * 2 + 32) + 2 * (AB_QB / 2) * (nk * 2 + 32);
+}
+inline bool attn_bwd_res_ok(int nk, int d, int dv) { return d == 32 && dv <= 128 && attn_bwd_res_lds(nk, d, dv) <= 160 * 1024; }
+
+__global__ __launch_bounds__(256) void attn_bwd_res_kernel(const bf16* __restrict__ q, const bf16* __restrict__ k,
+                                                           const bf16* __restrict__ v, const bf16* __restrict__ dout,
+                                                           const float* __restrict__ lse, bf16* __restrict__ dq,
+                                                           float* __restrict__ dk, float* __restrict__ dv, int N, int NK, int DV, int R) {
+    extern __shared__ __attribute__((aligned(16))) char bsm[];
+    constexpr int D = 32, ND = D / 32, PK = D * 2 + 32, HQ = AB_QB / 2, NDB = D / 16;
+    const int PDO = DV * 2 + 32, PP = NK * 2 + 32, PVL = DV * 2 + 16;
+    char* Ksm = bsm;
+    char* Vsm = Ksm + NK * PK;
+    char* Qsm = Vsm + NK * PVL;
+    char* dOsm = Qsm + AB_QB * PK;
+    char* Psm = dOsm + AB_QB * PDO;
+    char* dSsm = Psm + HQ * PP;
+    const int tid = threadIdx.x, lane = tid & 63, wave = tid >> 6;
+    const int b = blockIdx.y;
+    const int nqb = (N + AB_QB - 1) / AB_QB;
+    const int blk0 = blockIdx.x * R, nit = min(R, nqb - blk0);
+    const int i16 = lane & 15, g = lane >> 4;
+    const int ql = wave * 16 + i16;
+    const int nf = NK / 16, ncb = DV / 16;
+    const int cpq = D / 8, cpo = DV / 8;
+    const bf16* qimg = q + (long)b * N * D;
+    const bf16* doimg = dout + (long)b * N * DV;
+    const float* limg = lse + (long)b * N;
+    float l_cur = limg[min(blk0 * AB_QB + ql, N - 1)];
+    {
+        const int live = min(AB_QB, N - blk0 * AB_QB);
+        stage_chunks<8>(Ksm, PK, k + (long)b * NK * D, NK * cpq, NK * cpq, cpq, tid);
+        stage_chunks<8>(Vsm, PVL, v + (long)b * NK * DV, NK * cpo, NK * cpo, cpo, tid);
+        stage_chunks<ND>(Qsm, PK, qimg + (long)blk0 * AB_QB * D, AB_QB * cpq, live * cpq, cpq, tid);
+        stage_chunks<4>(dOsm, PDO, doimg + (long)blk0 * AB_QB * DV, AB_QB * cpo, live * cpo, cpo, tid);
+    }
+    f32x4_t accv[4][8], acck[4][NDB];
+#pragma unroll
+    for (int a = 0; a < 4; ++a) {
+#pragma unroll
+        for (int cb = 0; cb < 8; ++cb) accv[a][cb] = f32x4_t{0.f, 0.f, 0.f, 0.f};
+#pragma unroll
+        for (int db = 0; db < NDB; ++db) acck[a][db] = f32x4_t{0.f, 0.f, 0.f, 0.f};
+    }
+    const int rowsel = g * 4 + (i16 >> 2), colsel = (i16 & 3) * 8;
+    auto contract = [&](int h) {
+        uint4 pb[4], sb[4];
+#pragma unroll
+        for (int a = 0; a < 4; ++a) {
+            const int kf = wave + 4 * a, off = rowsel * PP + colsel + (kf < nf ? kf : 0) * 32;
+            pb[a] = tr_pair(Psm + off, 16 * PP);
+            sb[a] = tr_pair(dSsm + off, 16 * PP);
+        }
+#pragma unroll
+        for (int cb = 0; cb < 8; ++cb)
+            if (cb < ncb) {
+                const uint4 da = tr_pair(dOsm + (h * HQ + rowsel) * PDO + colsel + cb * 32, 16 * PDO);
+#pragma unroll
+                for (int a = 0; a < 4; ++a)
+                    accv[a][cb] = __builtin_amdgcn_mfma_f32_16x16x32_bf16(__builtin_bit_cast(bf16x8_t, da), __builtin_bit_cast(bf16x8_t, pb[a]), accv[a][cb], 0, 0, 0);
+            }
+#pragma unroll
+        for (int db = 0; db < NDB; ++db) {
+            const uint4 qa = tr_pair(Qsm + (h * HQ + rowsel) * PK + colsel + db * 32, 16 * PK);
+#pragma unroll
+            for (int a = 0; a < 4; ++a)
+                acck[a][db] = __builtin_amdgcn_mfma_f32_16x16x32_bf16(__builtin_bit_cast(bf16x8_t, qa), __builtin_bit_cast(bf16x8_t, sb[a]), acck[a][db], 0, 0, 0);
+        }
+    };
+    for (int it = 0; it < nit; ++it) {
+        const int qb0 = (blk0 + it) * AB_QB;
+        const bool q_ok = qb0 + ql < N;
+        __syncthreads();
+        f32x4_t pfr[AM_NKMAX / 16], dpf[AM_NKMAX / 16];
+#pragma unroll
+        for (int f = 0; f < AM_NKMAX / 16; ++f) { pfr[f] = f32x4_t{0.f, 0.f, 0.f, 0.f}; dpf[f] = f32x4_t{0.f, 0.f, 0.f, 0.f}; }
+#pragma unroll
+        for (int d0 = 0; d0 < D; d0 += 32) {
+            const uint4 qv = *reinterpret_cast<const uint4*>(Qsm + ql * PK + (d0 + g * 8) * 2);
+#pragma unroll
+            for (int f = 0; f < AM_NKMAX / 16; ++f)
+                if (f < nf) {
+                    const uint4 kv = *reinterpret_cast<const uint4*>(Ksm + (f * 16 + i16) * PK + (d0 + g * 8) * 2);
+                    pfr[f] = __builtin_amdgcn_mfma_f32_16x16x32_bf16(__builtin_bit_cast(bf16x8_t, kv), __builtin_bit_cast(bf16x8_t, qv), pfr[f], 0, 0, 0);
+                }
+        }
+        for (int c0 = 0; c0 < DV; c0 += 32) {
+            const uint4 dov = *reinterpret_cast<const uint4*>(dOsm + ql * PDO + (c0 + g * 8) * 2);
+#pragma unroll
+            for (int f = 0; f < AM_NKMAX / 16; ++f)
+                if (f < nf) {
+                    const uint4 vv = *reinterpret_cast<const uint4*>(Vsm + (f * 16 + i16) * PVL + (c0 + g * 8) * 2);
+                    dpf[f] = __builtin_amdgcn_mfma_f32_16x16x32_bf16(__builtin_bit_cast(bf16x8_t, vv), __builtin_bit_cast(bf16x8_t, dov), dpf[f], 0, 0, 0);
+                }
+        }
+        const float l = q_ok ? l_cur : 0.f;
+        float drow = 0.f;
+#pragma unroll
+        for (int f = 0; f < AM_NKMAX / 16; ++f)
+            if (f < nf) {
+#pragma unroll
+                for (int r = 0; r < 4; ++r) {
+                    const float pv = q_ok ? __expf(pfr[f][r] - l) : 0.f;
+                    pfr[f][r] = pv;
+                    drow += pv * dpf[f][r];
+                }
+            }
+        drow += __shfl_xor(drow, 16, 64);
+        drow += __shfl_xor(drow, 32, 64);
+        uint2 pw[AM_NKMAX / 16], sw[AM_NKMAX / 16];
+#pragma unroll
+        for (int f = 0; f < AM_NKMAX / 16; ++f) {
+            pw[f] = make_uint2(0, 0);
+            sw[f] = make_uint2(0, 0);
+            if (f < nf) {
+                pw[f].x = f32x2_to_bf16x2(pfr[f][0], pfr[f][1]);
+                pw[f].y = f32x2_to_bf16x2(pfr[f][2], pfr[f][3]);
+                sw[f].x = f32x2_to_bf16x2(pfr[f][0] * (dpf[f][0] - drow), pfr[f][1] * (dpf[f][1] - drow));
+                sw[f].y = f32x2_to_bf16x2(pfr[f][2] * (dpf[f][2] - drow), pfr[f][3] * (dpf[f][3] - drow));
+            }
+        }
+        {
+            f32x4_t dqa[NDB];
+#pragma unroll
+            for (int db = 0; db < NDB; ++db) dqa[db] = f32x4_t{0.f, 0.f, 0.f, 0.f};
+#pragma unroll
+            for (int t = 0; t < AM_NKMAX / 32; ++t)
+                if (t * 32 < NK) {
+                    const uint4 sb = make_uint4(sw[2 * t].x, sw[2 * t].y, sw[2 * t + 1].x, sw[2 * t + 1].y);
+                    const char* krow = Ksm + (t * 32 + g * 4 + (i16 >> 2)) * PK + (i16 & 3) * 8;
+#pragma unroll
+                    for (int db = 0; db < NDB; ++db) {
+                        const uint4 ka = tr_pair(krow + db * 32, 16 * PK);
+                        dqa[db] = __builtin_amdgcn_mfma_f32_16x16x32_bf16(__builtin_bit_cast(bf16x8_t, ka), __builtin_bit_cast(bf16x8_t, sb), dqa[db], 0, 0, 0);
+                    }
+                }
+            if (q_ok) {
+                bf16* qp = dq + ((long)b * N + qb0 + ql) * D + g * 4;
+#pragma unroll
+                for (int db = 0; db < NDB; ++db) {
+                    const float t4[4] = {dqa[db][0], dqa[db][1], dqa[db][2], dqa[db][3]};
+                    Elem<bf16>::st4(qp + db * 16, t4);
+                }
+            }
+        }
+        const bool more = it + 1 < nit;
+        const int live = more ? min(AB_QB, N - qb0 - AB_QB) : 1;
+        uint4 qn[ND], don[4];
+        float l_next = 0.f;
+        if (more) {
+            const uint4* q4 = reinterpret_cast<const uint4*>(qimg + (long)(qb0 + AB_QB) * D);
+            const uint4* o4 = reinterpret_cast<const uint4*>(doimg + (long)(qb0 + AB_QB) * DV);
+#pragma unroll
+            for (int i = 0; i < ND; ++i) qn[i] = q4[min(tid + i * 256, live * cpq - 1)];
+#pragma unroll
+            for (int i = 0; i < 4; ++i) don[i] = o4[min(tid + i * 256, live * cpo - 1)];
+            l_next = limg[min(qb0 + AB_QB + ql, N - 1)];
+        }
+        auto put = [&](int row) {
+#pragma unroll
+            for (int f = 0; f < AM_NKMAX / 16; ++f)
+                if (f < nf) {
+                    *reinterpret_cast<uint2*>(Psm + row * PP + (f * 16 + g * 4) * 2) = pw[f];
+                    *reinterpret_cast<uint2*>(dSsm + row * PP + (f * 16 + g * 4) * 2) = sw[f];
+                }
+        };
+        if (wave < 2) put(ql);
+        __syncthreads();
+        contract(0);
+        __syncthreads();
+        if (wave >= 2) put(ql - HQ);
+        __syncthreads();
+        contract(1);
+        if (more) {
+            __syncthreads();
+#pragma unroll
+            for (int i = 0; i < ND; ++i) {
+                const int e = tid + i * 256, row = e / cpq, c = e - row * cpq;
+                *reinterpret_cast<uint4*>(Qsm + row * PK + c * 16) = e < live * cpq ? qn[i] : make_uint4(0, 0, 0, 0);
+            }
+#pragma unroll
+            for (int i = 0; i < 4; ++i) {
+                const int e = tid + i * 256, row = e / cpo, c = e - row * cpo;
+                if (e < AB_QB * cpo) *reinterpret_cast<uint4*>(dOsm + row * PDO + c * 16) = e < live * cpo ? don[i] : make_uint4(0, 0, 0, 0);
+            }
+            l_cur = l_next;
+        }
+    }
+    float* dk_slab = dk + ((long)blockIdx.x * gridDim.y + b) * NK * D;
+    float* dv_slab = dv + ((long)blockIdx.x * gridDim.y + b) * NK * DV;
+#pragma unroll
+    for (int a = 0; a < 4; ++a) {
+        const int kf = wave + 4 * a;
+        if (kf < nf) {
+            float* dst = dv_slab + (long)(kf * 16 + i16) * DV + g * 4;
+#pragma unroll
+            for (int cb = 0; cb < 8; ++cb)
+                if (cb < ncb) *reinterpret_cast<float4*>(dst + cb * 16) = make_float4(accv[a][cb][0], accv[a][cb][1], accv[a][cb][2], accv[a][cb][3]);
+            dst = dk_slab + (long)(kf * 16 + i16) * D + g * 4;
+#pragma unroll
+            for (int db = 0; db < NDB; ++db)
+                *reinterpret_cast<float4*>(dst + db * 16) = make_float4(acck[a][db][0], acck[a][db][1], acck[a][db][2], acck[a][db][3]);
+        }
+    }
+}
+
+template <typename T>
+__global__ void attn_reduce2_kernel(const float* __restrict__ s0, long n0, T* __restrict__ d0, int blocks0,
+                                    const float* __restrict__ s1, long n1, T* __restrict__ d1, int nslabs) {
+    const bool first = (int)blockIdx.x < blocks0;
+    const float* src = first ? s0 : s1;
+    const long n = first ? n0 : n1;
+    T* dst = first ? d0 : d1;
+    const long i = (long)(first ? blockIdx.x : blockIdx.x - blocks0) * 256 + threadIdx.x;
+    if (i >= n / 4) return;
+    float4 a = reinterpret_cast<const float4*>(src)[i];
+    for (int s = 1; s < nslabs; s += 4) {
+        float4 t[4];
+#pragma unroll
+        for (int j = 0; j < 4; ++j) t[j] = reinterpret_cast<const float4*>(src + (long)min(s + j, nslabs - 1) * n)[i];
+#pragma unroll
+        for (int j = 0; j < 4; ++j)
+            if (s + j < nslabs) { a.x += t[j].x; a.y += t[j].y; a.z += t[j].z; a.w += t[j].w; }
+    }
+    const float o[4] = {a.x, a.y, a.z, a.w};
+    Elem<T>::st4(dst + i * 4, o);
 }
 
 template <typename T>
@@ -542,10 +846,18 @@
     SP_CHECK_ARG(nk > 0 && nk <= 256 && d > 0 && d <= 64 && dv > 0 && dv <= 256, "sp_attention_fwd: unsupported extents nk=%d d=%d dv=%d", nk, d, dv);
     hipStream_t s = reinterpret_cast<hipStream_t>(stream);
     if (attn_fwd_mfma_ok(dtype, nk, d, dv)) {
-        const int lds = nk * (dv * 2 + 32);
-        if (const int rc = sp_lds_limit<attn_fwd_mfma_kernel>(lds)) return rc;
-        hipLaunchKernelGGL(attn_fwd_mfma_kernel, dim3(sp_div_up(n, 64), batch), dim3(256), lds, s, (const bf16*)q, (const bf16*)k, (const bf16*)v,
-                           (bf16*)o, lse, n, nk, d, dv);
+        const int lds = attn_fwd_lds(nk, dv), nqb = sp_div_up(n, AB_QB);
+        const int walk = attn_walk(batch, nqb, attn_fwd_slots(attn_cus(), nk, dv), sp_tune(SP_TUNE_ATTN_PIECES, -1));
+        const dim3 grid(sp_div_up(nqb, walk), batch);
+        if (d == 32) {
+            if (const int rc = sp_lds_limit<attn_fwd_mfma_kernel<true>>(lds)) return rc;
+            hipLaunchKernelGGL(attn_fwd_mfma_kernel<true>, grid, dim3(256), lds, s, (const bf16*)q, (const bf16*)k, (const bf16*)v,
+                               (bf16*)o, lse, n, nk, d, dv, walk);
+        } else {
+            if (const int rc = sp_lds_limit<attn_fwd_mfma_kernel<false>>(lds)) return rc;
+            hipLaunchKernelGGL(attn_fwd_mfma_kernel<false>, grid, dim3(256), lds, s, (const bf16*)q, (const bf16*)k, (const bf16*)v,
+                               (bf16*)o, lse, n, nk, d, dv, walk);
+        }
         SP_LAUNCH_CHECK();
         return SP_OK;
     }
@@ -562,12 +874,31 @@
     const long nkd = (long)batch * nk * d, nkv = (long)batch * nk * dv;
     if (attn_bwd_mfma_ok(dtype, nk, d, dv)) {
         const int nqb = sp_div_up(n, AB_QB);
-        const int lds = nk * (d * 2 + 32) + AB_QB * (d * 2 + 32) + AB_QB * (dv * 2 + 32) + 2 * AB_QB * (nk * 2 + 32);
-        if (const int rc = sp_lds_limit<attn_bwd_mfma_kernel>(lds)) return rc;
-        hipLaunchKernelGGL(attn_bwd_mfma_kernel, dim3(nqb, batch), dim3(256), lds, s, (const bf16*)q, (const bf16*)k,
-                           (const bf16*)v, (const bf16*)dout, lse, (bf16*)dq, dk_f32, dv_f32, n, nk, d, dv);
-        hipLaunchKernelGGL(attn_reduce_kernel<bf16>, dim3(sp_div_up(nkd / 4, 256)), dim3(256), 0, s, dk_f32, nqb, nkd, (bf16*)dk);
-        hipLaunchKernelGGL(attn_reduce_kernel<bf16>, dim3(sp_div_up(nkv / 4, 256)), dim3(256), 0, s, dv_f32, nqb, nkv, (bf16*)dv_out);
+        int slabs = nqb;
+        if (sp_tune(SP_TUNE_ATTN_PIECES, -1) >= ATTN_TIMING_BIT) {
+            const int lds = nk * (d * 2 + 32) + AB_QB * (d * 2 + 32) + AB_QB * (dv * 2 + 32) + 2 * AB_QB * (nk * 2 + 32);
+            if (const int rc = sp_lds_limit<attn_bwd_mfma_kernel<true>>(lds)) return rc;
+            hipLaunchKernelGGL(attn_bwd_mfma_kernel<true>, dim3(nqb, batch), dim3(256), lds, s, (const bf16*)q, (const bf16*)k,
+                               (const bf16*)v, (const bf16*)dout, lse, (bf16*)dq, dk_f32, dv_f32, n, nk, d, dv);
+            SP_LAUNCH_CHECK();
+            return SP_OK;
+        }
+        if (attn_bwd_res_ok(nk, d, dv)) {
+            const int lds = attn_bwd_res_lds(nk, d, dv);
+            const int walk = attn_walk(batch, nqb, attn_cus(), sp_tune(SP_TUNE_ATTN_PIECES, -1));
+            slabs = sp_div_up(nqb, walk);
+            if (const int rc = sp_lds_limit<attn_bwd_res_kernel>(lds)) return rc;
+            hipLaunchKernelGGL(attn_bwd_res_kernel, dim3(slabs, batch), dim3(256), lds, s, (const bf16*)q, (const bf16*)k,
+                               (const bf16*)v, (const bf16*)dout, lse, (bf16*)dq, dk_f32, dv_f32, n, nk, dv, walk);
+        } else {
+            const int lds = nk * (d * 2 + 32) + AB_QB * (d * 2 + 32) + AB_QB * (dv * 2 + 32) + 2 * AB_QB * (nk * 2 + 32);
+            if (const int rc = sp_lds_limit<attn_bwd_mfma_kernel<false>>(lds)) return rc;
+            hipLaunchKernelGGL(attn_bwd_mfma_kernel<false>, dim3(nqb, batch), dim3(256), lds, s, (const bf16*)q, (const bf16*)k,
+                               (const bf16*)v, (const bf16*)dout, lse, (bf16*)dq, dk_f32, dv_f32, n, nk, d, dv);
+        }
+        const int blocks0 = sp_div_up(nkd / 4, 256);
+        hipLaunchKernelGGL(attn_reduce2_kernel<bf16>, dim3(blocks0 + sp_div_up(nkv / 4, 256)), dim3(256), 0, s, dk_f32, nkd, (bf16*)dk, blocks0,
+                           dv_f32, nkv, (bf16*)dv_out, slabs);
         SP_LAUNCH_CHECK();
         return SP_OK;
     }
@@ -593,6 +924,17 @@
     return SP_OK;
 }
 
+extern "C" int sp_attention_plan(int32_t batch, int32_t n, int32_t nk, int32_t d, int32_t dv, int32_t dtype, int32_t cus,
+                                 int32_t* fwd_walk, int32_t* bwd_walk, int32_t* bwd_slabs) {
+    SP_CHECK_ARG(fwd_walk && bwd_walk && bwd_slabs, "sp_attention_plan: null argument");
+    SP_CHECK_ARG(batch > 0 && n > 0 && nk > 0 && nk <= 256 && d > 0 && d <= 64 && dv > 0 && dv <= 256, "sp_attention_plan: unsupported extents batch=%d n=%d nk=%d d=%d dv=%d", batch, n, nk, d, dv);
+    const int nqb = sp_div_up(n, AB_QB), c = cus > 0 ? cus : attn_cus(), pieces = sp_tune(SP_TUNE_ATTN_PIECES, -1);
+    *fwd_walk = attn_fwd_mfma_ok(dtype, nk, d, dv) ? attn_walk(batch, nqb, attn_fwd_slots(c, nk, dv), pieces) : 0;
+    *bwd_walk = attn_bwd_mfma_ok(dtype, nk, d, dv) && attn_bwd_res_ok(nk, d, dv) ? attn_walk(batch, nqb, c, pieces) : 0;
+    *bwd_slabs = *bwd_walk ? sp_div_up(nqb, *bwd_walk) : attn_bwd_mfma_ok(dtype, nk, d, dv) ? nqb : sp_div_up(n, attn_valu_tq(nk, d, dv));
+    return SP_OK;
+}
+
 extern "C" int sp_attention_route(int32_t n, int32_t nk, int32_t d, int32_t dv, int32_t dtype, const char** fwd, const char** bwd) {
     SP_CHECK_ARG(fwd != nullptr && bwd != nullptr, "sp_attention_route: null argument");
     SP_CHECK_ARG(dtype == SP_F32 || dtype == SP_BF16, "sp_attention_route: unsupported storage type %d", dtype);
```
